# engcang/FAST-LIO-SAM-QN

Hardware: AMD Instinct MI355X
Metric: scan-pair registrations/sec on 100k-pt clouds (higher is better)
Workload: dtype f32 search / f64 accumulate

## Files before the change

### fast-lio-sam-qn_amd/csrc/qn_batch.inc

```

namespace {

template <class F> void lanes_launch(const void* tab, dim3 grid, hipStream_t s) {
  hipLaunchKernelGGL(HIP_KERNEL_NAME(k_lanes<F>), grid, dim3(F::TB), 0, s, (const LaneEntry<typename F::Args>*)tab);
}
template <class A> void lane_push(std::vector<LaneEntry<A>>& v, const A& a, uint32_t nbx) {
  LaneEntry<A> e; memset((void*)&e, 0, sizeof(e)); e.a = a; e.nbx = nbx; v.push_back(e);
}

struct LanePlan {
  qn_ctx* c; size_t off = 0; bool overflow = false; int flush_rc = QN_OK;
  struct Item { void (*fn)(const void*, dim3, hipStream_t); size_t off; dim3 grid; int family; };
  std::vector<Item> items;
  explicit LanePlan(qn_ctx* c_) : c(c_) {}
  template <class F> void add(const std::vector<LaneEntry<typename F::Args>>& e, int family) {
    if (e.empty()) return;
    const size_t bytes = sizeof(LaneEntry<typename F::Args>) * e.size();
    const size_t a = reserve(bytes);
    if (a == SIZE_MAX) return;
    put<F>(e, a, family);
  }
  template <class F, class Fix> void add(std::vector<LaneEntry<typename F::Args>>& e, int family, const void* blob, size_t blob_bytes, Fix fix) {
    if (e.empty()) return;
    const size_t head = (blob_bytes + 255) & ~(size_t)255, bytes = head + sizeof(LaneEntry<typename F::Args>) * e.size();
    const size_t a = reserve(bytes);
    if (a == SIZE_MAX) return;
    memcpy(c->args_h + a, blob, blob_bytes);
    fix(e, (const char*)(c->args_d + a));
    put<F>(e, a + head, family);
  }
  template <class F> void put(const std::vector<LaneEntry<typename F::Args>>& e, size_t a, int family) {
    const size_t bytes = sizeof(LaneEntry<typename F::Args>) * e.size();
    memcpy(c->args_h + a, e.data(), bytes);
    uint32_t gx = 0; for (const auto& x : e) gx = std::max(gx, x.nbx);
    gx = (gx + 7u) & ~7u;
    items.push_back(Item{&lanes_launch<F>, a, dim3(gx, (uint32_t)e.size()), family});
    off = a + bytes;
  }
  size_t reserve(size_t bytes) {
    size_t a = (off + 255) & ~(size_t)255;
    if (a + bytes > c->args_cap) {
      if (items.empty() || bytes > c->args_cap || flush_rc != QN_OK) { overflow = true; return SIZE_MAX; }
      flush_rc = run();
      if (flush_rc == QN_OK && hipStreamSynchronize(c->stream) != hipSuccess) { c->last_error = "batch: stream synchronisation failed while flushing the argument arena"; flush_rc = QN_ERR_HIP; }
      if (flush_rc != QN_OK) { overflow = true; return SIZE_MAX; }
      a = 0;
    }
    return a;
  }
  int run() {
    if (overflow) { if (flush_rc == QN_OK) c->last_error = "batch: argument arena too small for one launch's table"; return QN_ERR_HIP; }
    if (items.empty()) return QN_OK;
    HIPCHK(c, hipMemcpyAsync(c->args_d, c->args_h, off, hipMemcpyHostToDevice, c->stream));
    for (const Item& it : items) { c->prof_begin(it.family, (int)it.grid.y); it.fn(c->args_d + it.off, it.grid, c->stream); c->prof_end(); }
    c->batch_launches += items.size();
    items.clear(); off = 0;
    HIPCHK(c, hipGetLastError());
    return QN_OK;
  }
};

struct ScratchSwap {
  qn_ctx* c;
  static void sw(qn_ctx* c) {
    std::swap(c->scan_sums, c->scan_sums2); std::swap(c->fb_list, c->fb_list2); std::swap(c->big_list, c->big_list2); std::swap(c->fb_count2, c->fb_count2b);
    std::swap(c->knn_idx, c->knn_idx2); std::swap(c->bbox_acc, c->bbox_acc2); std::swap(c->scan_status, c->scan_status2); std::swap(c->staging, c->staging2); std::swap(c->pin_up, c->pin_up2);
  }
  explicit ScratchSwap(qn_ctx* c_) : c(c_) { sw(c); }
  ~ScratchSwap() { sw(c); }
};

struct LaneRun {
  qn_ctx* c = nullptr; uint32_t pair = 0; bool active = false;
  int alias = -1;
  int ticks_left = 0, chunk = 0, chunk_start = 0, next = 0; bool first_chunk = true; long budget = 0;
  bool build_source = true;
};

int lane_set_cloud(qn_ctx* c, int which, const float* xyz, uint32_t n, uint32_t stride, bool on_device, hipStream_t s, GridLaunch* out) {
  CloudBuf& b = c->cloud[which];
  b.n = 0; b.has_grid = b.has_cov = false;
  if (n == 0) return QN_ERR_EMPTY_CLOUD;
  if (!xyz || stride < 12 || (stride & 3)) return QN_ERR_INVALID_ARG;
  if (n > c->max_points) return QN_ERR_CAPACITY;
  const char* dsrc = (const char*)xyz;
  if (!on_device) { const int rc = upload_host_cloud(c, xyz, n, stride, s, &dsrc); if (rc != QN_OK) return rc; }
  b.n = n;
  *out = prep_grid(c, b, dsrc, stride, true);
  return QN_OK;
}

bool batch_supported(const qn_ctx* c) {
  const qn_gicp_params& p = c->params;
  const int maxit = p.force_iterations > 0 ? p.force_iterations : p.max_iterations;
  return c->knob.batch_lanes >= 2 && !c->lanes_failed && maxit > 0 && c->knob.far_enabled && c->knob.knn_hist && !c->knob.verify_track && !c->clk_probe && !c->list_probe && !c->dbg_counters;
}

int lane_args_arena(qn_ctx* c) {
  if (c->args_h) return QN_OK;
  c->args_cap = (size_t)4 << 20;
  HIPCHK(c, hipHostMalloc(&c->args_h, c->args_cap, hipHostMallocDefault));
  HIPCHK(c, hipMalloc(&c->args_d, c->args_cap));
  return QN_OK;
}

int batch_ensure_lanes(qn_ctx* c) {
  HIPCHK(c, hipSetDevice(c->device));
  const int B = std::max(1, std::min(c->knob.batch_lanes, 64));
  if (c->lanes.empty()) c->lanes.push_back(c);
  while ((int)c->lanes.size() < B) {
    qn_ctx* l = nullptr;
    const int rc = (c->knob.fail_lane_create > 0 && (int)c->lanes.size() >= c->knob.fail_lane_create) ? QN_ERR_HIP : ctx_create(c->device, c->max_points, c->stream, &l);
    if (rc != QN_OK) {
      c->last_error = "batch: lane context creation failed (lanes need batch_lanes x the context's device memory)";
      while (c->lanes.size() > 1) { qn_ctx_destroy(c->lanes.back()); c->lanes.pop_back(); }
      (void)hipGetLastError();
      c->lanes_failed = true;
      return rc;
    }
    c->lanes.push_back(l);
  }
  { const int rc = lane_args_arena(c); if (rc != QN_OK) return rc; }
  for (qn_ctx* l : c->lanes) {
    if (l == c) continue;
    if (l->params.k_correspondences != c->params.k_correspondences) l->cloud[0].has_cov = l->cloud[1].has_cov = false;
    l->params = c->params;
    l->lane = c->lane;
  }
  return QN_OK;
}

int batch_register(qn_ctx* owner, const qn_pair_desc* pairs, const uint32_t* idx, uint32_t m, double thr, qn_gicp_result* results, int* valid, int* status,
                   std::vector<const float*>& last_src, std::vector<uint64_t>& last_key, const float* guesses16) {
  hipStream_t s = owner->stream;
  const auto t_call = std::chrono::steady_clock::now();
  const qn_gicp_params& p = owner->params;
  const int k = p.k_correspondences;
  LanePlan plan(owner);
  std::vector<LaneRun> L(m);
  struct AliasGuard {
    std::vector<LaneRun>& L; std::vector<CloudBuf> saved; std::vector<double*> saved_nrm; std::vector<const float*>& last_src;
    AliasGuard(std::vector<LaneRun>& L_, std::vector<const float*>& ls) : L(L_), saved(L_.size()), saved_nrm(L_.size(), nullptr), last_src(ls) {}
    void borrow(size_t l, qn_ctx* from) { qn_ctx* c = L[l].c; saved[l] = c->cloud[0]; saved_nrm[l] = c->nrm_s_sorted; c->cloud[0] = from->cloud[0]; c->nrm_s_sorted = from->nrm_s_sorted; }
    ~AliasGuard() { for (size_t l = 0; l < L.size(); l++) if (L[l].alias >= 0 && saved_nrm[l]) { qn_ctx* c = L[l].c; c->cloud[0] = saved[l]; c->nrm_s_sorted = saved_nrm[l]; c->cloud[0].has_grid = c->cloud[0].has_cov = false; c->cloud[0].n = 0; c->cloud[0].knn_tab = nullptr; last_src[l] = nullptr; } }
  } alias_guard(L, last_src);
  struct FailGuard { std::vector<LaneRun>& L; int* status; bool armed = true; ~FailGuard() { if (armed) for (const LaneRun& R : L) if (R.active) status[R.pair] = QN_ERR_HIP; } } fail_guard{L, status};
  std::vector<LaneEntry<PackBBoxK::Args>> v_pack; std::vector<LaneEntry<CellCountK::Args>> v_count; std::vector<LaneEntry<ScanLookbackK::Args>> v_scan;
  std::vector<LaneEntry<ScatterK::Args>> v_scat; std::vector<LaneEntry<StableCellsK::Args>> v_stab;
// ... 23 lines not shown
      if (R.alias >= 0) { alias_guard.borrow(l, L[R.alias].c); R.build_source = false; }
    }
    int rc = QN_OK; GridLaunch gs, gt;
    if (R.build_source) { last_src[l] = nullptr; rc = lane_set_cloud(c, QN_SOURCE, pd.src, pd.ns, pd.stride_bytes, pd.on_device != 0, s, &gs); }
    if (rc == QN_OK) { ScratchSwap sw(c); rc = lane_set_cloud(c, QN_TARGET, pd.dst, pd.nt, pd.stride_bytes, pd.on_device != 0, s, &gt); }
    if (rc == QN_ERR_HIP) return rc;
    status[R.pair] = rc;
    if (rc != QN_OK) {
      if (R.build_source) { c->cloud[0].has_grid = c->cloud[0].has_cov = false; c->cloud[0].n = 0; }
      c->cloud[1].has_grid = c->cloud[1].has_cov = false; c->cloud[1].n = 0;
      continue;
    }
    if (R.build_source) { push_grid(gs); push_knn(prep_knn(c, c->cloud[0], k, c->knn_idx, nullptr, true)); c->cloud[0].has_cov = true; note_knn_table(c, c->cloud[0], c->knn_idx, k); }
    { ScratchSwap sw(c); push_grid(gt); push_knn(prep_knn(c, c->cloud[1], k, c->knn_idx, nullptr, true)); c->cloud[1].has_cov = true; note_knn_table(c, c->cloud[1], c->knn_idx, k); }
    last_src[l] = R.alias >= 0 ? nullptr : pd.src; last_key[l] = key;
    R.active = true;
  }
  plan.add<PackBBoxK>(v_pack, QN_K_GRID_BUILD); plan.add<CellCountK>(v_count, QN_K_GRID_BUILD); plan.add<ScanLookbackK>(v_scan, QN_K_GRID_BUILD); plan.add<ScatterK>(v_scat, QN_K_GRID_BUILD); plan.add<StableCellsK>(v_stab, QN_K_GRID_BUILD);
  if (k <= 24) {
    if (owner->lane.knn_mm) { plan.add<KnnHistK<false, 32>>(v_sel, QN_K_KNN_SELECT); plan.add<KnnHistK<true, 32>>(v_lst, QN_K_KNN_COV); }
    else { plan.add<KnnHistK<false, 32, false>>(v_sel, QN_K_KNN_SELECT); plan.add<KnnHistK<true, 32, false>>(v_lst, QN_K_KNN_COV); }
  } else {
    if (owner->lane.knn_mm) { plan.add<KnnHistK<false, 48>>(v_sel, QN_K_KNN_SELECT); plan.add<KnnHistK<true, 48>>(v_lst, QN_K_KNN_COV); }
    else { plan.add<KnnHistK<false, 48, false>>(v_sel, QN_K_KNN_SELECT); plan.add<KnnHistK<true, 48, false>>(v_lst, QN_K_KNN_COV); }
  }
  plan.add<KnnSingleK>(v_single, QN_K_KNN_COV);
  if (k <= 16) plan.add<KnnCovK<16, true, 4>>(v_tail, QN_K_KNN_COV); else if (k <= 20) plan.add<KnnCovK<20, true, 4>>(v_tail, QN_K_KNN_COV); else if (k <= 24) plan.add<KnnCovK<24, true, 4>>(v_tail, QN_K_KNN_COV); else plan.add<KnnCovK<32, true, 4>>(v_tail, QN_K_KNN_COV);
  plan.add<CovFromIdxK>(v_cov, QN_K_KNN_COV);

  const int per_outer = p.optimizer == QN_OPT_LM ? 2 : 1;
  const int maxit = p.force_iterations > 0 ? p.force_iterations : p.max_iterations;
  const int fixed_unseeded = fixed_unseeded_iterations(owner) * per_outer;
  const bool exact_ticks = p.force_iterations > 0 && p.optimizer == QN_OPT_GN;
  {
    std::vector<LaneEntry<InitStateK::Args>> v_init; std::vector<float> g16;
    for (LaneRun& R : L) {
      if (!R.active) continue;
      qn_ctx* c = R.c;
      c->gen = 0; c->part_rows = 0; c->far_mode = 2; c->clear_far_now = true; c->unseeded_until = fixed_unseeded; c->count_far_now = false;
      c->result_host->phase = 0;
      R.ticks_left = exact_ticks ? maxit : 1 << 30;
      R.chunk = std::min(fixed_unseeded, R.ticks_left); R.chunk_start = 0; R.next = R.chunk; R.first_chunk = true;
      R.budget = (long)maxit * (p.optimizer == QN_OPT_LM ? (p.lm_max_iterations + 1) : 1) + 2;
      lane_push(v_init, InitStateK::Args{st_cur(c), c->guess_tmp, guesses16 ? 1 : 0, 0, c->far_stats}, 1u);
      if (guesses16) g16.insert(g16.end(), guesses16 + 16 * (size_t)R.pair, guesses16 + 16 * (size_t)R.pair + 16);
    }
    if (!guesses16) plan.add<InitStateK>(v_init, QN_K_SOLVE);
    else
      plan.add<InitStateK>(v_init, QN_K_SOLVE, g16.data(), sizeof(float) * g16.size(), [](std::vector<LaneEntry<InitStateK::Args>>& e, const char* d) {
        for (size_t j = 0; j < e.size(); j++) e[j].a.guess = (const float*)(d + sizeof(float) * 16 * j);
      });
  }
  auto finish_lane = [&](LaneRun& R, int rc) {
    qn_ctx* c = R.c;
    R.active = false;
    status[R.pair] = rc;
    if (rc != QN_OK) return;
    results[R.pair] = c->result_host->r;
    c->trace_len = c->result_host->trace_len; c->aligned_valid = true;
    valid[R.pair] = (results[R.pair].converged && results[R.pair].fitness < thr) ? 1 : 0;
  };
  struct ProfFlush { qn_ctx* c; ~ProfFlush() { c->prof_collect(); } } prof_flush{owner};
  int tick_no = 0;
  for (;;) {
    int stop = 1 << 30; bool any = false;
    for (const LaneRun& R : L) if (R.active) { any = true; stop = std::min(stop, R.next); }
    if (!any) break;
    for (; tick_no < stop; tick_no++) {
      {
        std::vector<LaneEntry<NnSearchArgs>> v_g, v_l; std::vector<LaneEntry<AccumulateK::Args>> v_acc;
        bool group = true, lane = true;
        for (LaneRun& R : L) {
          if (!R.active || tick_no >= R.c->unseeded_until) continue;
          qn_ctx* c = R.c;
          const int t = tick_no - R.chunk_start;
          c->count_far_now = R.first_chunk && (t / per_outer == (R.chunk - 1) / per_outer);
          const NnLaunch N = prep_nn(c, 0, c->sqd, 0);
          group = group && N.group; lane = lane && N.lane;
          lane_push(v_g, N.grid, N.grid_nb); lane_push(v_l, N.list, N.list_nb);
          const uint32_t nb = acc_blocks(c);
          lane_push(v_acc, prep_accumulate(c, 0, true), nb);
          c->count_far_now = false;
        }
        if (lane) plan.add<NnLaneK<0>>(v_g, QN_K_NN_SEARCH); else plan.add<NnSearchK<0, false, QN_NN_BLOCK>>(v_g, QN_K_NN_SEARCH);
        if (group) plan.add<NnSearchK<0, true, QN_BLOCK, true>>(v_l, QN_K_NN_FALLBACK); else plan.add<NnSearchK<0, true, QN_BLOCK>>(v_l, QN_K_NN_FALLBACK);
        plan.add<AccumulateK>(v_acc, QN_K_ACCUMULATE);
      }
      {
        std::vector<LaneEntry<TickArgs>> v_t; std::vector<LaneEntry<FarArgs>> v_f; std::vector<LaneEntry<FarReduceK::Args>> v_r;
        for (LaneRun& R : L) {
          if (!R.active || tick_no < R.c->unseeded_until) continue;
          qn_ctx* c = R.c;
          const TickArgs a = tick_args(c);
          lane_push(v_t, a, tick_blocks(c));
          if (a.far_mode == 1) { lane_push(v_f, far_args(c), (uint32_t)QN_FAR_BLOCKS); lane_push(v_r, far_reduce_args(c), 1u); }
          c->gen++; c->part_rows = -1;
        }
        plan.add<TickK<TICK_TB, 4, 0, false>>(v_t, QN_K_GN_TICK_FUSED); plan.add<FarK>(v_f, QN_K_FAR); plan.add<FarReduceK>(v_r, QN_K_FAR);
      }
    }
    {
      std::vector<LaneEntry<FinalizeK::Args>> v_fin; std::vector<LaneEntry<TickArgs>> v_close; std::vector<LaneEntry<FinalizeFitK::Args>> v_fit;
      for (LaneRun& R : L) {
        if (!R.active || R.next != stop) continue;
        qn_ctx* c = R.c;
        if (exact_ticks && R.ticks_left > R.chunk) lane_push(v_fin, FinalizeK::Args{st_cur(c), c->result_host, c->far_stats}, 1u);
        else {
          const TickArgs a = tick_args(c, 1);
          const uint32_t nb = tick_blocks(c);
          lane_push(v_close, a, nb);
          lane_push(v_fit, FinalizeFitK::Args{st_cur(c), c->result_host, c->far_stats, c->fit_psum, c->fit_pcnt, (int)tick_rows(c)}, 1u);
        }
      }
      plan.add<FinalizeK>(v_fin, QN_K_SOLVE); plan.add<TickK<TICK_TB, 4, 1, false>>(v_close, QN_K_FITNESS); plan.add<FinalizeFitK>(v_fit, QN_K_FITNESS);
    }
    const auto tt0 = std::chrono::steady_clock::now();
    int rc = plan.run();
    if (rc != QN_OK) return rc;
    const auto tt1 = std::chrono::steady_clock::now();
    HIPCHK(owner, hipStreamSynchronize(s));
    if (owner->knob.batch_trace) { const auto tt2 = std::chrono::steady_clock::now();
      fprintf(stderr, "qn batch %p: segment to tick %d  prep+enqueue %.0f us  sync %.0f us  (since call %.0f us)\n", (void*)owner, stop, std::chrono::duration<double, std::micro>(tt1 - tt0).count(),
              std::chrono::duration<double, std::micro>(tt2 - tt1).count(), std::chrono::duration<double, std::micro>(tt2 - t_call).count()); }
    for (LaneRun& R : L) {
      if (!R.active || R.next != stop) continue;
      qn_ctx* c = R.c;
      if (R.first_chunk && (rc = clouds_valid(c)) != QN_OK) { last_src[&R - &L[0]] = nullptr; finish_lane(R, rc); continue; }
      R.budget -= std::max(R.chunk, 1); R.ticks_left -= R.chunk;
      if (c->result_host->phase == 2) { finish_lane(R, QN_OK); continue; }
      if (R.budget <= 0) { c->last_error = "align: device state machine did not terminate"; owner->last_error = c->last_error; finish_lane(R, QN_ERR_HIP); continue; }
      if (R.first_chunk && unseeded_goes_on(c, stop, per_outer, R.ticks_left)) {
        c->unseeded_until = stop + per_outer; R.chunk = per_outer; R.chunk_start = stop; R.next = stop + R.chunk;
        continue;
      }
      const qn::ResultBlock* rb = c->result_host;
      if (R.first_chunk) c->far_mode = rb->far_queries * 16u > c->cloud[0].n ? 1 : 2;
      else c->far_mode = (c->far_mode == 1 ? rb->far_requests : rb->far_misses / (uint32_t)std::max(1, R.chunk)) > 256u ? 1 : 2;
      if (!exact_ticks) R.chunk = R.first_chunk ? TICKS_PER_CHUNK : std::max(2 * per_outer, TICKS_PER_CHUNK / 2);
      else R.chunk = c->far_mode == 1 ? std::min(R.ticks_left, FAR_CHUNK) : R.ticks_left;
      if (R.budget <= 0 || R.chunk <= 0) { c->last_error = "align: device state machine did not terminate"; owner->last_error = c->last_error; finish_lane(R, QN_ERR_HIP); continue; }
      R.first_chunk = false; R.chunk_start = stop; R.next = stop + R.chunk;
    }
  }
  owner->batch_pairs += m;
  fail_guard.armed = false;
  return QN_OK;
}

}

extern "C" int qn_gicp_align_batch_guess(qn_ctx* c, const qn_pair_desc* pairs, const float* guesses16, uint32_t n_pairs, double score_thr, qn_gicp_result* results, int* valid, int* status) {
  if (!c || (n_pairs && (!pairs || !results || !valid || !status))) return QN_ERR_INVALID_ARG;
  if (guesses16)
    for (uint32_t i = 0; i < n_pairs; i++) {
      const float* g = guesses16 + 16 * (size_t)i;
      for (int j = 0; j < 16; j++) if (!std::isfinite(g[j])) { c->last_error = "align_batch_guess: non-finite guess entry"; return QN_ERR_INVALID_ARG; }
      if (g[12] != 0.f || g[13] != 0.f || g[14] != 0.f || g[15] != 1.f) { c->last_error = "align_batch_guess: a guess's last row is not 0 0 0 1"; return QN_ERR_INVALID_ARG; }
    }
  if (n_pairs == 0) return QN_OK;
  HIPCHK(c, hipSetDevice(c->device));
  if (join_target(c) != QN_OK) return QN_ERR_HIP;
  int rc = batch_supported(c) ? batch_ensure_lanes(c) : QN_ERR_NOT_READY;
  if (rc != QN_OK) {
    const bool sp = c->knob.pair_pipeline, sb = c->knob.persist_batch_off; c->knob.pair_pipeline = false; c->knob.persist_batch_off = true;
    for (uint32_t i = 0; i < n_pairs; i++) {
      const qn_pair_desc& p = pairs[i];
// ... 24 lines not shown
```

### fast-lio-sam-qn_amd/csrc/qn_context.h

```cpp
#pragma once
#include <hip/hip_runtime.h>
#include <string>
#include <vector>
#include "qn_gicp_kernels.cuh"

struct CloudBuf {
  uint32_t n = 0, ncells = 0;
  bool has_grid = false, has_cov = false;
  float4* raw = nullptr;
  float4* sorted = nullptr;
  float4* sorted_tmp = nullptr;
  uint32_t* cell_of_pt = nullptr;
  uint32_t* cell_start = nullptr;
  uint32_t* counts = nullptr;
  double* nrm = nullptr;
  qn::GridView grid{};
  qn::GridDims* dims = nullptr;
  qn::GridDims* dims_host = nullptr;
  const int32_t* knn_tab = nullptr; int knn_k = 0;
};

struct ProfSpan { int family; hipEvent_t a, b; int count; };

struct LaneKnobs {
  double cell_override = 0.0;
  int far_group = -1;
  bool far_ranked = true;
  int nn_lane = -1;
  int track_from_tick = 3;
  int knn_mm = 1;
  int knn_trips = 3;
  uint32_t tick_rpb = 2;
};
struct FeatKnobs {
  bool mfma = true;
  int sample = 4;
  bool query_dedupe = false;
  int normals_fg = 0, fpfh_fg = 0;
};
struct OwnKnobs {
  bool device_look = true;
  int single_from_tick = 2;
  bool far_enabled = true;
  int knn_hist = 1;
  bool tgt_early = true;
  bool pair_pipeline = true;
  bool persist = true, prof_persist = false; unsigned long long persist_timeout = 25000000ull;
  bool persist_batch_off = false;
  int batch_lanes = 8;
  int fail_lane_create = 0;
  bool batch_share_source = true;
  bool batch_trace = false;
  int batch_min_share = 4;
  bool c2f_lanes_fpfh = false;
  bool feat_verify = false;
  bool verify_track = false;
};

struct qn_ctx {
  int device = 0;
  uint32_t max_points = 0, max_cells = 0;
  hipStream_t stream = nullptr; bool owns_stream = true;
  LaneKnobs lane; FeatKnobs feat; OwnKnobs knob;
  std::vector<qn_ctx*> lanes; char* args_h = nullptr; char* args_d = nullptr; size_t args_cap = 0; uint64_t batch_launches = 0, batch_pairs = 0; bool is_lane = false;
  bool lanes_failed = false;
  void* slab = nullptr;
  qn_gicp_params params{};
  CloudBuf cloud[2];
  qn::BBoxAcc* bbox_acc = nullptr; qn::BBoxAcc* bbox_acc2 = nullptr;
  unsigned long long* scan_status = nullptr; unsigned long long* scan_status2 = nullptr; uint32_t build_epoch = 0;
  unsigned long long* list_probe = nullptr;
  bool clear_far_now = false;
  char* staging2 = nullptr;
  struct PinZone { char* h = nullptr; hipEvent_t ev = nullptr; bool busy = false; } pin_up, pin_up2;
  char* staging = nullptr;
  uint32_t* scan_sums = nullptr;

  qn::GicpState* state = nullptr;
  uint32_t gen = 0; int part_rows = 0;
  double* partials = nullptr;
  uint32_t* tail_ticket = nullptr;
  double* fit_psum = nullptr; uint32_t* fit_pcnt = nullptr;
  qn_iter_trace* trace = nullptr; uint32_t trace_len = 0;
  int32_t* corr = nullptr; int32_t* nn_idx = nullptr; int32_t* knn_idx = nullptr; float4* nn_ref = nullptr; double* nrm_s_sorted = nullptr; qn::TargetRec* tgt_rec = nullptr; float* sqd = nullptr; float* sqd_fit = nullptr;
  int32_t* far_cand = nullptr; float4* far_cand_ref = nullptr; float2* far_cand_b = nullptr; unsigned long long* far_req = nullptr; uint32_t* far_stats = nullptr; double* far_rows = nullptr; int far_mode = 2;
  uint2* fb_list = nullptr; uint2* big_list = nullptr; uint32_t* fb_count2 = nullptr;
  float4* aligned = nullptr; bool aligned_valid = false;
  double* pose_tmp = nullptr; float* guess_tmp = nullptr;
  qn::ResultBlock* result_host = nullptr; double* scalar_host = nullptr;
  int32_t* dbg_knn_idx = nullptr; float* dbg_knn_d2 = nullptr;
  qn_quatro_params qparams{}; bool qparams_set = false, q_ready = false; double q_last_scale = 1.0;
  float4* q_normals[2] = {nullptr, nullptr}; float* q_spfh[2] = {nullptr, nullptr}; float* q_fpfh_s[2] = {nullptr, nullptr}; float* q_fpfh[2] = {nullptr, nullptr};
  unsigned long long* q_key[2] = {nullptr, nullptr};
  float* q_pair[2] = {nullptr, nullptr}; uint32_t* q_pair_hash[2] = {nullptr, nullptr};
  uint32_t* q_hit = nullptr; uint32_t* q_list = nullptr; uint32_t* q_sel = nullptr; uint2* q_pairs = nullptr; uint32_t* q_counts = nullptr; double* q_T = nullptr;
  void* q_mm_c = nullptr; void* q_mm_q = nullptr; float* q_mm_qn = nullptr; uint32_t* q_mm_L = nullptr; unsigned long long* q_mm_table = nullptr; unsigned long long* q_mm_table_q = nullptr;
  uint32_t q_mm_mask = 0;
  uint2* q_mm_pairs = nullptr; uint32_t* q_mm_cnt = nullptr; uint32_t q_mm_cap = 0, q_mm_ncnt = 0; bool feat_mm_retry = false; double q_wall_ms[3] = {0, 0, 0}; unsigned long long* q_mm_vkeys = nullptr; uint32_t* q_mm_vcnt = nullptr; uint32_t feat_fallbacks = 0, feat_survivors = 0;
  float4* c2f_src = nullptr; float4* c2f_dst = nullptr;
  float* q_mean = nullptr; double* q_mean_psum = nullptr; void* q_host = nullptr;
  int unseeded_until = 3; bool count_far_now = false; int last_extra_unseeded = 0;
  hipStream_t stream2 = nullptr; hipEvent_t ev_pair = nullptr; bool pair_failed = false, tgt_on_stream2 = false, tgt_pending = false, no_pipe = false;
  uint32_t* scan_sums2 = nullptr; uint2* fb_list2 = nullptr; uint2* big_list2 = nullptr; uint32_t* fb_count2b = nullptr; int32_t* knn_idx2 = nullptr;
  unsigned long long* pg_rows = nullptr; unsigned long long* pg_bc = nullptr; unsigned long long* pg_fit = nullptr; uint32_t* pg_status = nullptr; uint32_t* pg_status_host = nullptr;
  unsigned long long* pg_clk = nullptr; uint32_t pg_epoch = 0; bool persist_fits = true; int persist_resident_blocks = 0; uint32_t persist_launches = 0, persist_gave_up = 0;
  uint32_t* dbg_counters = nullptr;
  unsigned long long* clk_probe = nullptr; uint32_t clk_n = 0;
  int32_t* v_corr = nullptr; int32_t* v_nn_idx = nullptr; float* v_sqd = nullptr; float4* v_nn_ref = nullptr; uint32_t* v_counters = nullptr;
  bool prof_on = false, prof_open = false; int prof_depth = 0;
  std::vector<ProfSpan> spans;
  qn_kernel_stat stats[QN_K_COUNT] = {};
  std::string last_error;

  void set_error(const char* what, hipError_t e, int line);
  void prof_begin(int family, int count = 1); void prof_end(); void prof_collect();
  int quatro_normals_width() const { const int g = feat.normals_fg > 0 ? feat.normals_fg : 8; return g >= 16 ? 16 : (g >= 8 ? 8 : 1); }
  int quatro_fpfh_width() const { const int g = feat.fpfh_fg > 0 ? feat.fpfh_fg : 8; return g >= 16 ? 16 : 8; }
};
```

### fast-lio-sam-qn_amd/csrc/qn_device.cuh

```cuda
#pragma once
#include <hip/hip_runtime.h>
#include <stdint.h>
#include "qn_eig3.cuh"
#include "qn_step_math.cuh"

namespace qn {

#define QN_TX 8
#define QN_TY 4
#define QN_TZ 4
#define QN_TILE_CELLS 128

struct GridDims {
  float ox, oy, oz, cell, inv_cell, eps;
  int nx, ny, nz, ntx, nty, ntz;
  uint32_t n;
  uint32_t ncells, nonfinite, pad;
};
struct GridView {
  const float4* pts;
  const uint32_t* cell_start;
  uint32_t* dbg;
  float ox, oy, oz, cell, inv_cell, eps;
  int nx, ny, nz;
// ... 437 lines not shown
  for (uint32_t cb = 0; cb < total; cb += 64) {
    const uint32_t slot = cb + lane;
    const int j = chunk_segment(lds->tile_cid, cb, ex, nxs);
    const uint32_t cnt = min(64u, total - cb);
    wave_lds_fence();
    lds->tile[lane] = slot < total ? g.pts[lds->seg_start[j] + (slot - lds->seg_excl[j])] : make_float4(INF, INF, INF, 0.f);
    lds->tile_cid[lane] = slot < total ? lds->seg_cid[j] : 0xffffffffu;
    wave_lds_fence();
    const uint32_t sub_off = (uint32_t)(S == 1 ? 0 : lane / (64 / S));
    for (uint32_t c = 0; c < cnt; c += 4 * S) {
      float4 cp[4]; uint32_t cc[4];
#pragma unroll
      for (int u = 0; u < 4; u++) { const uint32_t ci = (c + (uint32_t)(S * u) + sub_off) & 63u; cp[u] = lds->tile[ci]; cc[u] = lds->tile_cid[ci]; }
#pragma unroll
      for (int u = 0; u < 4; u++) fn(cp[u], true, cc[u]);
    }
  }
}
template <bool REUSE = false, class Chunks>
__device__ __forceinline__ uint32_t stream_tables(const GridView& g, WaveLds* lds, int ncl, uint32_t nseg_all, Chunks&& chunks, const uint32_t reuse_total = 0) {
  const int lane = threadIdx.x & 63;
  if (REUSE && nseg_all <= 64u) { chunks(reuse_total); return reuse_total; }
  uint32_t ncand = 0;
  for (uint32_t sb = 0; sb < nseg_all; sb += 64) {
    const uint32_t sidx = sb + lane;
    uint32_t s = 0, len = 0, scid = 0;
    if (sidx < nseg_all) {
      int c = 0;
#pragma unroll
      for (int step = 32; step > 0; step >>= 1) { const int t = c + step; if (t < ncl && lds->cl_seg0[t] <= sidx) c = t; }
      const int* b = lds->box[c];
      const int x0 = b[0], x1 = b[1], y0 = b[2], y1 = b[3], z0 = b[4];
      const int tx0 = x0 >> 3, ntr = (x1 >> 3) - tx0 + 1;
      const int li = (int)(sidx - lds->cl_seg0[c]);
      int t, rr; divmod_small(li, ntr, rr, t);
      if (lds->cl_tile_mode[c]) {
        const int ty0 = y0 >> 2, ntyr = (y1 >> 2) - ty0 + 1;
        int qz_, ry_; divmod_small(rr, ntyr, qz_, ry_);
        const uint32_t tile = ((uint32_t)((z0 >> 2) + qz_) * g.nty + (ty0 + ry_)) * g.ntx + (tx0 + t);
        s = g.cell_start[tile << 7]; len = g.cell_start[(tile + 1) << 7] - s;
      } else {
        const int nyr = y1 - y0 + 1;
        int qz_, ry_; divmod_small(rr, nyr, qz_, ry_);
        const int ry = y0 + ry_, rz = z0 + qz_, tx = tx0 + t;
        const int xa = max(x0, tx << 3), xb = min(x1, (tx << 3) + 7);
        const uint32_t k0 = cell_key(g, xa, ry, rz);
        s = g.cell_start[k0]; len = g.cell_start[k0 + (xb - xa) + 1] - s;
      }
      scid = (uint32_t)c;
    }
    const uint32_t incl = wave_incl_scan_u32(len, lane);
    const uint32_t total = rdlane(incl, 63);
    if (total == 0) continue;
    wave_lds_fence();
    lds->seg_excl[lane] = incl - len; lds->seg_start[lane] = s; lds->seg_cid[lane] = scid;
    wave_lds_fence();
    chunks(total);
    ncand += total;
  }
  return ncand;
}
template <int S, bool REUSE = false, class Fn>
__device__ __forceinline__ uint32_t stream_clusters(const GridView& g, WaveLds* lds, int ncl, uint32_t nseg_all, Fn&& fn, const uint32_t reuse_total = 0) {
  return stream_tables<REUSE>(g, lds, ncl, nseg_all, [&](const uint32_t total) __attribute__((always_inline)) { stream_chunks<S>(g, lds, total, fn); }, reuse_total);
}

template <int S, class Sink>
__device__ __forceinline__ bool wave_search(const GridView& g, float qx, float qy, float qz, bool active, float& r, const float r_cap,
                                            int max_rounds, Sink& sink, WaveLds* lds, float& d_unseen) {
  const int lane = threadIdx.x & 63;
  const int cx = cell_coord(qx, g.ox, g.inv_cell, g.nx);
  const int cy = cell_coord(qy, g.oy, g.inv_cell, g.ny);
  const int cz = cell_coord(qz, g.oz, g.inv_cell, g.nz);
  bool certified = false;
  unsigned long long todo = __ballot(active);
  for (int round = 0; todo != 0 && round < max_rounds; round++) {
    const bool mine = (todo >> lane) & 1ull;
    uint32_t cid; int ncl; uint32_t nseg_all;
    build_clusters<S>(g, lds, todo, cx, cy, cz, qx, qy, qz, r, cid, ncl, nseg_all);
    const uint32_t ncand = stream_clusters<S>(g, lds, ncl, nseg_all, [&](const float4& cp, bool in_tile, uint32_t ccid) __attribute__((always_inline)) {
      sink.consider(mine && in_tile && ccid == cid, sqdist(qx, qy, qz, cp.x, cp.y, cp.z), __float_as_uint(cp.w));
    });
    sink.template finish<S>(mine);
    if (g.dbg && lane == 0) { atomicAdd(&g.dbg[0], (uint32_t)ncl); atomicAdd(&g.dbg[1], ncand); }
    bool retry = false;
    if (mine) {
      const int* b = lds->box[cid];
      const int ex0 = b[0], ex1 = b[1], ey0 = b[2], ey1 = b[3], ez0 = b[4], ez1 = b[5];
      const float INF = __int_as_float(0x7f800000);
      float d = INF;
      if (ex0 > 0) d = fminf(d, qx - (g.ox + ex0 * g.cell));
      if (ex1 < g.nx - 1) d = fminf(d, (g.ox + (ex1 + 1) * g.cell) - qx);
      if (ey0 > 0) d = fminf(d, qy - (g.oy + ey0 * g.cell));
      if (ey1 < g.ny - 1) d = fminf(d, (g.oy + (ey1 + 1) * g.cell) - qy);
      if (ez0 > 0) d = fminf(d, qz - (g.oz + ez0 * g.cell));
      if (ez1 < g.nz - 1) d = fminf(d, (g.oz + (ez1 + 1) * g.cell) - qz);
      if (d == INF || !(r == r)) { certified = true; d_unseen = INF; }
      else { d -= g.eps; d_unseen = d; certified = d > 0.f && sink.full() && sink.worst_d2() < d * d; }
      if (!certified) {
        if (sink.full()) r = fmaxf(sqrtf(sink.worst_d2()) * 1.000001f + g.eps, r + g.eps);
        else {
          const int f = sink.found();
          r = f > 0 ? fmaxf(r * sqrtf((float)sink.wanted() / (float)f) * 1.25f, r + g.cell) : 2.f * r + g.cell;
        }
        r = fminf(r, r_cap);
        if (round + 1 < max_rounds) { retry = true; sink.reset(); }
      }
    }
    todo = __ballot(retry);
    if (g.dbg && lane == 0 && todo) atomicAdd(&g.dbg[3], (uint32_t)__popcll(todo));
  }
  return certified;
}

struct CapBox {
  float o2[3];
  float S;
};
__device__ __forceinline__ CapBox cap_of(const GridView& g, float qx, float qy, float qz) {
  CapBox c;
  const float ox = fmaxf(fmaxf(g.ox - qx, qx - (g.ox + g.nx * g.cell)), 0.f);
  const float oy = fmaxf(fmaxf(g.oy - qy, qy - (g.oy + g.ny * g.cell)), 0.f);
  const float oz = fmaxf(fmaxf(g.oz - qz, qz - (g.oz + g.nz * g.cell)), 0.f);
  c.o2[0] = ox * ox; c.o2[1] = oy * oy; c.o2[2] = oz * oz; c.S = (c.o2[0] + c.o2[1]) + c.o2[2];
  return c;
}
__device__ __forceinline__ float cap_extent(const GridView& g, const CapBox& c, float r, int axis) {
  const float rest = c.S - c.o2[axis];
  if (rest <= 0.f) return r;
  const float v = r * r - rest * 0.999999f;
  return v > 0.f ? sqrtf(v) * 1.000001f + g.eps : g.eps;
}
__device__ __forceinline__ float cap_face_dist(const CapBox& c, float f, int axis) {
  const float rest = (c.S - c.o2[axis]) * 0.999999f;
  return rest > 0.f ? sqrtf(f * f + rest) * 0.999999f : f;
}

struct SingleStats { uint32_t rounds, cand, segs; float r_first, r_last; };
__device__ __forceinline__ void wave_search_single(const GridView& g, float qx, float qy, float qz, float r, const float r_cap,
                                                   unsigned long long& best_out, float& second_out, float& d_unseen, WaveLds* lds, SingleStats& st_out, const bool stats) {
  const int lane = threadIdx.x & 63;
  const float INF = __int_as_float(0x7f800000);
  const CapBox cap = cap_of(g, qx, qy, qz);
  if (cap.S > 0.f) r = fminf(fmaxf(r, sqrtf(cap.S) + g.cell), fmaxf(r_cap, r));
  if (stats) { st_out.rounds = 0; st_out.cand = 0; st_out.segs = 0; st_out.r_first = r; }
  float done2 = -1.f;
  int ptx0 = 0, ptx1 = -1, pty0 = 0, pty1 = -1, ptz0 = 0, ptz1 = -1;
  unsigned long long best = QN_INF_KEY; float second = INF;
  for (int round = 0;; round++) {
    const float rx = cap_extent(g, cap, r, 0), ry = cap_extent(g, cap, r, 1), rz = cap_extent(g, cap, r, 2);
    int x0 = rfl(cell_coord(qx - rx, g.ox, g.inv_cell, g.nx)), x1 = rfl(cell_coord(qx + rx, g.ox, g.inv_cell, g.nx));
    int y0 = rfl(cell_coord(qy - ry, g.oy, g.inv_cell, g.ny)), y1 = rfl(cell_coord(qy + ry, g.oy, g.inv_cell, g.ny));
    int z0 = rfl(cell_coord(qz - rz, g.oz, g.inv_cell, g.nz)), z1 = rfl(cell_coord(qz + rz, g.oz, g.inv_cell, g.nz));
    const int tx0 = x0 >> 3, ntr = (x1 >> 3) - tx0 + 1;
    int nseg = ntr * (y1 - y0 + 1) * (z1 - z0 + 1);
    const bool tile_mode = nseg > 128;
    int ty0 = 0, ntyr = 1;
    if (tile_mode) {
      x0 = (x0 >> 3) << 3; x1 = min(((x1 >> 3) << 3) + 7, g.nx - 1);
      y0 = (y0 >> 2) << 2; y1 = min(((y1 >> 2) << 2) + 3, g.ny - 1);
      z0 = (z0 >> 2) << 2; z1 = min(((z1 >> 2) << 2) + 3, g.nz - 1);
      ty0 = y0 >> 2; ntyr = (y1 >> 2) - ty0 + 1;
      nseg = ntr * ntyr * ((z1 >> 2) - (z0 >> 2) + 1);
    }
    const int nyr = y1 - y0 + 1;
    if (!tile_mode || done2 < 0.f) { best = QN_INF_KEY; second = INF; done2 = -1.f; }
    const float in2 = r * r * 1.000002f;
// ... 205 lines not shown
```

### fast-lio-sam-qn_amd/csrc/qn_engine.hip

```cpp
#include <hip/hip_runtime.h>
#include <cfloat>
#include <cmath>
#include <cstdio>
#include <cstring>
#include <string>
#include <vector>
#include <atomic>
#include <thread>
#include <chrono>
#include "qn_instances.h"
#include "qn_context.h"
#include "qn_selftest.cuh"
#include "qn_pool.h"
#include "qn_kf_internal.h"

using namespace qn;

#define HIPCHK(ctx, call)                                                                 \
  do { hipError_t e_ = (call);                                                            \
       if (e_ != hipSuccess) { (ctx)->set_error(#call, e_, __LINE__); return QN_ERR_HIP; } \
  } while (0)

void qn_ctx::set_error(const char* what, hipError_t e, int line) {
  char buf[512]; snprintf(buf, sizeof(buf), "%s -> %s (qn_engine.hip:%d)", what, hipGetErrorString(e), line);
// ... 30 lines not shown
    case QN_OK: return "ok"; case QN_ERR_INVALID_ARG: return "invalid argument"; case QN_ERR_EMPTY_CLOUD: return "empty cloud";
    case QN_ERR_CAPACITY: return "cloud exceeds context capacity"; case QN_ERR_NOT_READY: return "clouds/covariances not set";
    case QN_ERR_HIP: return "HIP runtime error"; case QN_ERR_NO_DEVICE: return "no gfx950 device (no CPU fallback)";
    case QN_ERR_INTERNAL: return "internal error (a bounded loop left its bound)";
  }
  return "unknown status";
}
extern "C" const char* qn_last_error(const qn_ctx* ctx) { return ctx ? ctx->last_error.c_str() : "null context"; }

extern "C" void qn_gicp_default_params(qn_gicp_params* p) {
  if (!p) return;
  memset(p, 0, sizeof(*p));
  p->k_correspondences = 20; p->max_iterations = 64; p->max_corr_dist = (double)FLT_MAX;
  p->transformation_epsilon = 5e-4; p->rotation_epsilon = 2e-3; p->optimizer = QN_OPT_LM;
  p->lm_max_iterations = 10; p->lm_init_lambda_factor = 1e-9; p->force_iterations = 0;
  p->ransac_iterations = 0; p->ransac_outlier_threshold = 0.05; p->euclidean_fitness_epsilon = -DBL_MAX;
}

struct Slab {
  char* base = nullptr; size_t off = 0, cap = 0;
  template <class T> void take(T*& p, size_t bytes) {
    const size_t a = (off + 255) & ~(size_t)255;
    if (base) p = (T*)(base + a);
    off = a + bytes;
  }
};
static void carve_cloud(qn_ctx* c, Slab& sl, CloudBuf& b) {
  sl.take(b.raw, sizeof(float4) * c->max_points);
  sl.take(b.sorted, sizeof(float4) * c->max_points);
  sl.take(b.sorted_tmp, sizeof(float4) * c->max_points);
  sl.take(b.cell_of_pt, sizeof(uint32_t) * c->max_points);
  sl.take(b.cell_start, sizeof(uint32_t) * ((size_t)c->max_cells + 1));
  sl.take(b.counts, sizeof(uint32_t) * ((size_t)c->max_cells + 1));
  sl.take(b.nrm, sizeof(double) * 3 * c->max_points);
  sl.take(b.dims, sizeof(GridDims));
}

static int ctx_create(int device, uint32_t max_points, hipStream_t shared_stream, qn_ctx** out);
extern "C" int qn_ctx_create(int device, uint32_t max_points, qn_ctx** out) { return ctx_create(device, max_points, nullptr, out); }
static int ctx_create(int device, uint32_t max_points, hipStream_t shared_stream, qn_ctx** out) {
  if (!out || max_points == 0) return QN_ERR_INVALID_ARG;
  *out = nullptr;
  if (max_points > QN_CTX_MAX_POINTS) return QN_ERR_CAPACITY;
  int ndev = 0;
  if (hipGetDeviceCount(&ndev) != hipSuccess || ndev <= 0 || device < 0 || device >= ndev) return QN_ERR_NO_DEVICE;
  qn_ctx* c = new qn_ctx();
  c->device = device; c->max_points = max_points;
  size_t mc = (size_t)max_points * 16; if (mc < (1u << 18)) mc = 1u << 18; if (mc > (1u << 23)) mc = 1u << 23;
  c->max_cells = (uint32_t)mc;
  qn_gicp_default_params(&c->params);
  int rc = QN_OK;
  auto fail = [&](int code) { qn_ctx_destroy(c); return code; };
  if (hipSetDevice(device) != hipSuccess) return fail(QN_ERR_NO_DEVICE);
  if (shared_stream) { c->stream = shared_stream; c->owns_stream = false; c->is_lane = true; }
  else if (hipStreamCreateWithFlags(&c->stream, hipStreamNonBlocking) != hipSuccess) return fail(QN_ERR_HIP);
#define CA(call) if ((call) != hipSuccess) return fail(QN_ERR_HIP)
  auto carve = [&](Slab& sl) {
    carve_cloud(c, sl, c->cloud[0]);
    carve_cloud(c, sl, c->cloud[1]);
    sl.take(c->staging, (size_t)max_points * 32);
    sl.take(c->scan_sums, sizeof(uint32_t) * (c->max_cells / (QN_BLOCK * QN_SCAN_ITEMS) + 2));
    sl.take(c->state, 2 * sizeof(GicpState));
    sl.take(c->partials, 2 * sizeof(double) * (QN_ACC_MAX_BLOCKS + 8) * QN_NPART);
    sl.take(c->nn_idx, sizeof(int32_t) * max_points);
    sl.take(c->knn_idx, sizeof(int32_t) * (size_t)max_points * 32);
    sl.take(c->nn_ref, sizeof(float4) * max_points);
    sl.take(c->nrm_s_sorted, sizeof(double) * 3 * max_points);
    sl.take(c->tgt_rec, sizeof(TargetRec) * max_points);
    sl.take(c->fit_psum, sizeof(double) * (QN_ACC_MAX_BLOCKS + 8));
    sl.take(c->fit_pcnt, sizeof(uint32_t) * (QN_ACC_MAX_BLOCKS + 8));
    sl.take(c->trace, sizeof(qn_iter_trace) * QN_MAX_TRACE);
    sl.take(c->corr, sizeof(int32_t) * max_points);
    sl.take(c->sqd, sizeof(float) * max_points);
    sl.take(c->sqd_fit, sizeof(float) * max_points);
    sl.take(c->far_cand, sizeof(int32_t) * QN_FAR_M * (size_t)max_points);
    sl.take(c->far_cand_ref, sizeof(float4) * max_points);
    sl.take(c->far_cand_b, sizeof(float2) * max_points);
    sl.take(c->far_req, sizeof(unsigned long long) * (max_points / 64 + 2));
    sl.take(c->far_stats, 4 * sizeof(uint32_t));
    sl.take(c->far_rows, sizeof(double) * QN_FAR_BLOCKS * QN_NPART);
    sl.take(c->fb_list, sizeof(uint2) * max_points);
    sl.take(c->big_list, sizeof(uint2) * max_points);
    sl.take(c->fb_count2, 4 * sizeof(uint32_t));
    sl.take(c->aligned, sizeof(float4) * max_points);
    sl.take(c->pose_tmp, sizeof(double) * 16);
    sl.take(c->guess_tmp, sizeof(float) * 16);
    sl.take(c->scan_sums2, sizeof(uint32_t) * (c->max_cells / (QN_BLOCK * QN_SCAN_ITEMS) + 2));
    sl.take(c->fb_list2, sizeof(uint2) * max_points);
    sl.take(c->big_list2, sizeof(uint2) * max_points);
    sl.take(c->fb_count2b, 4 * sizeof(uint32_t));
    sl.take(c->knn_idx2, sizeof(int32_t) * (size_t)max_points * 32);
    sl.take(c->staging2, (size_t)max_points * 32);
    sl.take(c->bbox_acc, 2 * (QN_BBOX_MAX_BLOCKS + 1) * sizeof(BBoxAcc)); c->bbox_acc2 = c->bbox_acc ? c->bbox_acc + (QN_BBOX_MAX_BLOCKS + 1) : nullptr;
    sl.take(c->scan_status, sizeof(unsigned long long) * 2 * (c->max_cells / (QN_BLOCK * QN_SCAN_ITEMS) + 2)); c->scan_status2 = c->scan_status ? c->scan_status + (c->max_cells / (QN_BLOCK * QN_SCAN_ITEMS) + 2) : nullptr;
    sl.take(c->pg_rows, sizeof(unsigned long long) * 3 * QN_PERSIST_ROWS * QN_PERSIST_RSTRIDE);
    sl.take(c->pg_bc, sizeof(unsigned long long) * 64);
    sl.take(c->pg_fit, sizeof(unsigned long long) * (QN_PERSIST_MAX_BLOCKS + 1) * 4);
    sl.take(c->pg_status, 4 * sizeof(uint32_t));
    sl.take(c->tail_ticket, 4 * sizeof(uint32_t));
  };
  { Slab dry; carve(dry);
    Slab sl; sl.cap = (dry.off + ((size_t)2 << 20) - 1) & ~(((size_t)2 << 20) - 1);
    CA(hipMalloc(&c->slab, sl.cap)); sl.base = (char*)c->slab; carve(sl); }
  CA(hipMemsetAsync(c->far_stats, 0, 4 * sizeof(uint32_t), c->stream));
  CA(hipHostMalloc(&c->result_host, sizeof(ResultBlock), hipHostMallocDefault));
  for (int w = 0; w < 2; w++) { CA(hipHostMalloc(&c->cloud[w].dims_host, sizeof(GridDims), hipHostMallocDefault)); memset(c->cloud[w].dims_host, 0, sizeof(GridDims)); }
  CA(hipHostMalloc(&c->scalar_host, 64 * sizeof(double), hipHostMallocDefault));
  CA(hipHostMalloc(&c->pg_status_host, 4 * sizeof(uint32_t), hipHostMallocDefault));
  CA(hipMemsetAsync(c->pg_rows, 0xFF, sizeof(unsigned long long) * 3 * QN_PERSIST_ROWS * QN_PERSIST_RSTRIDE, c->stream));
  CA(hipMemsetAsync(c->pg_bc, 0, sizeof(unsigned long long) * 64, c->stream));
  CA(hipMemsetAsync(c->pg_fit, 0, sizeof(unsigned long long) * (QN_PERSIST_MAX_BLOCKS + 1) * 4, c->stream));
  CA(hipMemsetAsync(c->pg_status, 0, 4 * sizeof(uint32_t), c->stream));
  CA(hipMemsetAsync(c->tail_ticket, 0, 4 * sizeof(uint32_t), c->stream));
  CA(hipMemsetAsync(c->state, 0, 2 * sizeof(GicpState), c->stream));
  hipLaunchKernelGGL(k_bbox_acc_init, dim3(1), dim3(256), 0, c->stream, c->bbox_acc, 2 * (QN_BBOX_MAX_BLOCKS + 1));
  CA(hipMemsetAsync(c->fb_count2, 0, 4 * sizeof(uint32_t), c->stream)); CA(hipMemsetAsync(c->fb_count2b, 0, 4 * sizeof(uint32_t), c->stream));
  CA(hipMemsetAsync(c->scan_status, 0, sizeof(unsigned long long) * 2 * (c->max_cells / (QN_BLOCK * QN_SCAN_ITEMS) + 2), c->stream));
  for (int w = 0; w < 2; w++) CA(hipMemsetAsync(c->cloud[w].counts, 0, sizeof(uint32_t) * ((size_t)c->max_cells + 1), c->stream));
  CA(hipMemsetAsync(c->knn_idx, 0xff, sizeof(int32_t) * (size_t)max_points * 32, c->stream));
  if (c->knn_idx2) CA(hipMemsetAsync(c->knn_idx2, 0xff, sizeof(int32_t) * (size_t)max_points * 32, c->stream));
  CA(hipStreamSynchronize(c->stream));
#undef CA
  {
    int per_cu = 0; hipDeviceProp_t prop;
    if (hipOccupancyMaxActiveBlocksPerMultiprocessor(&per_cu, reinterpret_cast<const void*>(&k_align_persist<QN_PERSIST_TB, false>), QN_PERSIST_TB, 0) != hipSuccess || hipGetDeviceProperties(&prop, device) != hipSuccess) { (void)hipGetLastError(); per_cu = 0; prop.multiProcessorCount = 0; }
    c->persist_resident_blocks = per_cu * prop.multiProcessorCount;
    c->persist_fits = c->persist_resident_blocks >= QN_PERSIST_MAX_BLOCKS + 1;
  }
  *out = c;
  return QN_OK;
}

extern "C" void qn_ctx_destroy(qn_ctx* c) {
  if (!c) return;
  hipSetDevice(c->device);
  if (c->stream) hipStreamSynchronize(c->stream);
  if (c->stream2) hipStreamSynchronize(c->stream2);
  for (qn_ctx* l : c->lanes) if (l != c) qn_ctx_destroy(l);
  c->lanes.clear();
  if (c->args_h) hipHostFree(c->args_h);
  hipFree(c->args_d);
  c->prof_collect();
  hipFree(c->slab);
  hipFree(c->q_mm_c); hipFree(c->q_mm_q); hipFree(c->q_mm_qn); hipFree(c->q_mm_L); hipFree(c->q_mm_table); hipFree(c->q_mm_table_q); hipFree(c->q_mm_pairs); hipFree(c->q_mm_cnt); hipFree(c->q_mm_vkeys); hipFree(c->q_mm_vcnt);
  for (int w = 0; w < 2; w++) { hipFree(c->q_normals[w]); hipFree(c->q_spfh[w]); hipFree(c->q_fpfh_s[w]); hipFree(c->q_fpfh[w]); hipFree(c->q_key[w]); hipFree(c->q_pair[w]); hipFree(c->q_pair_hash[w]); }
  hipFree(c->q_hit); hipFree(c->q_list); hipFree(c->q_sel); hipFree(c->q_pairs); hipFree(c->q_counts); hipFree(c->q_T); hipFree(c->q_mean); hipFree(c->q_mean_psum);
  if (c->q_host) hipHostFree(c->q_host);
  hipFree(c->c2f_src); hipFree(c->c2f_dst);
  hipFree(c->dbg_knn_idx); hipFree(c->dbg_knn_d2); hipFree(c->dbg_counters);
  hipFree(c->v_corr); hipFree(c->v_nn_idx); hipFree(c->v_sqd); hipFree(c->v_nn_ref); hipFree(c->v_counters);
  if (c->result_host) hipHostFree(c->result_host);
  for (int w = 0; w < 2; w++) if (c->cloud[w].dims_host) hipHostFree(c->cloud[w].dims_host);
  if (c->scalar_host) hipHostFree(c->scalar_host);
  hipFree(c->pg_clk); if (c->list_probe) hipFree(c->list_probe); if (c->pg_status_host) hipHostFree(c->pg_status_host);
  if (c->ev_pair) hipEventDestroy(c->ev_pair);
  for (qn_ctx::PinZone* z : {&c->pin_up, &c->pin_up2}) { if (z->ev) hipEventDestroy(z->ev); if (z->h) hipHostFree(z->h); }
  if (c->stream2) { hipStreamSynchronize(c->stream2); hipStreamDestroy(c->stream2); }
  if (c->stream && c->owns_stream) hipStreamDestroy(c->stream);
  delete c;
}

static int clouds_valid(qn_ctx* c);
extern "C" void* qn_ctx_stream(qn_ctx* c) { return c ? (void*)c->stream : nullptr; }
int qn_ctx_int_device(const qn_ctx* c) { return c->device; }
int qn_ctx_int_max_points(const qn_ctx* c) { return (int)c->max_points; }
extern "C" int qn_ctx_synchronize(qn_ctx* c) {
  if (!c) return QN_ERR_INVALID_ARG;
  HIPCHK(c, hipStreamSynchronize(c->stream));
  if (c->stream2) HIPCHK(c, hipStreamSynchronize(c->stream2));
  c->prof_collect();
  return clouds_valid(c);
}

extern "C" int qn_gicp_set_params(qn_ctx* c, const qn_gicp_params* p) {
  if (!c || !p) return QN_ERR_INVALID_ARG;
  if (p->k_correspondences < 1 || p->k_correspondences > 32 || p->max_iterations < 0 || p->lm_max_iterations < 1 ||
      (p->optimizer != QN_OPT_LM && p->optimizer != QN_OPT_GN) || !(p->max_corr_dist > 0) || !(p->lm_init_lambda_factor >= 0)) return QN_ERR_INVALID_ARG;
  if (p->k_correspondences != c->params.k_correspondences) { c->cloud[0].has_cov = c->cloud[1].has_cov = false; }
  c->params = *p;
  return QN_OK;
}

extern "C" int qn_gicp_get_params(const qn_ctx* c, qn_gicp_params* p) { if (!c || !p) return QN_ERR_INVALID_ARG; *p = c->params; return QN_OK; }

static GicpConfig make_cfg(const qn_ctx* c) {
  GicpConfig g; const qn_gicp_params& p = c->params;
  g.k = p.k_correspondences; g.max_iterations = p.max_iterations; g.optimizer = p.optimizer; g.lm_max_iterations = p.lm_max_iterations;
  g.force_iterations = p.force_iterations; g.max_corr_dist_sq = p.max_corr_dist * p.max_corr_dist;
  g.transformation_epsilon = p.transformation_epsilon; g.rotation_epsilon = p.rotation_epsilon; g.lm_init_lambda_factor = p.lm_init_lambda_factor;
  return g;
}

static inline GicpState* st_cur(qn_ctx* c) { return c->state + (c->gen & 1u); }
static inline GicpState* st_nxt(qn_ctx* c) { return c->state + ((c->gen + 1u) & 1u); }
static inline double* part_cur(qn_ctx* c) { return c->partials + (size_t)(c->gen & 1u) * (QN_ACC_MAX_BLOCKS + 8) * QN_NPART; }
static inline double* part_nxt(qn_ctx* c) { return c->partials + (size_t)((c->gen + 1u) & 1u) * (QN_ACC_MAX_BLOCKS + 8) * QN_NPART; }

static bool pair_pipeline_ready(qn_ctx* c) {
  if (c->stream2) return true;
  if (c->pair_failed || !c->knn_idx2) return false;
  const bool ok = hipStreamCreateWithFlags(&c->stream2, hipStreamNonBlocking) == hipSuccess && hipEventCreateWithFlags(&c->ev_pair, hipEventDisableTiming) == hipSuccess;
  if (!ok) { c->pair_failed = true; if (c->stream2) { hipStreamDestroy(c->stream2); c->stream2 = nullptr; } (void)hipGetLastError(); }
  return ok;
}
static void swap_scratch(qn_ctx* c) {
  std::swap(c->stream, c->stream2); std::swap(c->scan_sums, c->scan_sums2); std::swap(c->fb_list, c->fb_list2); std::swap(c->big_list, c->big_list2);
  std::swap(c->fb_count2, c->fb_count2b); std::swap(c->knn_idx, c->knn_idx2);
  std::swap(c->bbox_acc, c->bbox_acc2); std::swap(c->scan_status, c->scan_status2);
  std::swap(c->pin_up, c->pin_up2);
  std::swap(c->staging, c->staging2);
}
struct TargetScope {
  qn_ctx* c; bool on;
  TargetScope(qn_ctx* c_, bool on_) : c(c_), on(on_) { if (on) swap_scratch(c); }
  ~TargetScope() { if (on) { (void)hipEventRecord(c->ev_pair, c->stream); swap_scratch(c); c->tgt_pending = true; } }
};
static int join_target(qn_ctx* c) {
  if (!c->tgt_pending) return QN_OK;
  c->tgt_pending = false;
  return hipStreamWaitEvent(c->stream, c->ev_pair, 0) == hipSuccess ? QN_OK : QN_ERR_HIP;
}

struct GridLaunch { PackBBoxK::Args pack; uint32_t pack_nb; CellCountK::Args count; ScanLookbackK::Args scan; uint32_t scan_nb; ScatterK::Args scat; StableCellsK::Args stab; uint32_t nb; };
static GridLaunch prep_grid(qn_ctx* c, CloudBuf& b, const char* dsrc, uint32_t stride, bool lanes = false) {
  const uint32_t n = b.n;
  GridView& g = b.grid;
  memset(&g, 0, sizeof(g));
  g.pts = b.sorted; g.cell_start = b.cell_start; g.dbg = c->dbg_counters; g.n = n; g.dims = b.dims;
  GridLaunch L;
  L.nb = (n + QN_BLOCK - 1) / QN_BLOCK;
  L.scan_nb = (c->max_cells + QN_BLOCK * QN_SCAN_ITEMS - 1) / (QN_BLOCK * QN_SCAN_ITEMS);
  if (((++c->build_epoch) & 0x3fffffffu) == 0u) ++c->build_epoch;
  constexpr int LONE_PACK_BLOCKS = 64;
  static_assert(LONE_PACK_BLOCKS <= QN_BBOX_MAX_BLOCKS, "the accumulator has one box per block");
  L.pack_nb = std::min<uint32_t>(L.nb, (uint32_t)(lanes ? QN_BBOX_MAX_BLOCKS : LONE_PACK_BLOCKS));
  L.pack = PackBBoxK::Args{dsrc, stride, n, b.raw, c->bbox_acc, c->max_cells, c->lane.cell_override, b.dims, b.dims_host};
  L.count = CellCountK::Args{b.raw, n, g, b.counts, b.cell_of_pt};
  L.scan = ScanLookbackK::Args{b.counts, b.dims, b.cell_start, c->scan_status, c->build_epoch, n};
  L.scat = ScatterK::Args{b.raw, n, b.cell_of_pt, b.cell_start, b.counts, b.sorted_tmp};
  L.stab = StableCellsK::Args{b.sorted_tmp, n, b.cell_of_pt, b.cell_start, b.sorted};
  b.has_grid = true; b.has_cov = false; b.knn_tab = nullptr;
  return L;
}
static int build_grid(qn_ctx* c, CloudBuf& b, const char* dsrc, uint32_t stride) {
  hipStream_t s = c->stream;
  const GridLaunch L = prep_grid(c, b, dsrc, stride);
  { ProfScope ps(c, QN_K_GRID_BUILD);
    hipLaunchKernelGGL(k_pack_bbox_dims, dim3(L.pack_nb), dim3(QN_BLOCK), 0, s, L.pack.in, L.pack.stride, L.pack.n, L.pack.raw, L.pack.acc, L.pack.max_cells, L.pack.cell_override, L.pack.dims_dev, L.pack.dims_host);
    hipLaunchKernelGGL(k_cell_count, dim3(L.nb), dim3(QN_BLOCK), 0, s, L.count.pts, L.count.n, L.count.g, L.count.counts, L.count.cell_of_pt);
    hipLaunchKernelGGL(k_scan_lookback, dim3(L.scan_nb), dim3(QN_BLOCK), 0, s, L.scan.in, L.scan.dims, L.scan.out, L.scan.status, L.scan.epoch, L.scan.total);
    hipLaunchKernelGGL(k_scatter, dim3(L.nb), dim3(QN_BLOCK), 0, s, L.scat.pts, L.scat.n, L.scat.cell_of_pt, L.scat.cell_start, L.scat.counts, L.scat.sorted);
    hipLaunchKernelGGL(k_stable_cells, dim3(L.nb), dim3(QN_BLOCK), 0, s, L.stab.in, L.stab.n, L.stab.cell_of_pt, L.stab.cell_start, L.stab.out); }
  HIPCHK(c, hipGetLastError());
  return QN_OK;
}
static int clouds_valid(qn_ctx* c) {
  for (int w = 0; w < 2; w++)
    if (c->cloud[w].has_grid && c->cloud[w].dims_host && c->cloud[w].dims_host->nonfinite) {
      c->last_error = w == 0 ? "source cloud contains non-finite coordinates (is_dense == false clouds are not supported)" : "target cloud contains non-finite coordinates (is_dense == false clouds are not supported)";
      c->cloud[w].has_grid = c->cloud[w].has_cov = false;
      return QN_ERR_INVALID_ARG;
    }
  return QN_OK;
}

static int upload_host_cloud(qn_ctx* c, const float* xyz, uint32_t n, uint32_t& stride, hipStream_t s, const char** dsrc) {
  hipPointerAttribute_t at;
  const bool pinned = hipPointerGetAttributes(&at, xyz) == hipSuccess && at.type == hipMemoryTypeHost;
  if (!pinned) (void)hipGetLastError();
  if (pinned) {
    if (stride <= 32) { HIPCHK(c, hipMemcpyAsync(c->staging, xyz, (size_t)(n - 1) * stride + 12, hipMemcpyHostToDevice, s)); }
    else { HIPCHK(c, hipMemcpy2DAsync(c->staging, 16, xyz, stride, 16, n, hipMemcpyHostToDevice, s)); stride = 16; }
    *dsrc = (const char*)c->staging;
    return QN_OK;
  }
  qn_ctx::PinZone& z = c->pin_up;
  if (!z.h) { HIPCHK(c, hipHostMalloc((void**)&z.h, (size_t)c->max_points * 16, hipHostMallocDefault)); HIPCHK(c, hipEventCreateWithFlags(&z.ev, hipEventDisableTiming)); }
  if (z.busy) { HIPCHK(c, hipEventSynchronize(z.ev)); z.busy = false; }
  float* o = (float*)z.h; const char* in = (const char*)xyz;
  for (uint32_t i = 0; i < n; i++, in += stride, o += 3) { const float* p = (const float*)in; o[0] = p[0]; o[1] = p[1]; o[2] = p[2]; }
  HIPCHK(c, hipMemcpyAsync(c->staging, z.h, (size_t)n * 12, hipMemcpyHostToDevice, s));
  HIPCHK(c, hipEventRecord(z.ev, s)); z.busy = true;
  stride = 12; *dsrc = (const char*)c->staging;
  return QN_OK;
}

static int set_cloud(qn_ctx* c, int which, const float* xyz, uint32_t n, uint32_t stride, bool on_device) {
  if (!c || (which != 0 && which != 1)) return QN_ERR_INVALID_ARG;
  CloudBuf& b = c->cloud[which];
  b.n = 0; b.has_grid = b.has_cov = false;
// ... 33 lines not shown
  L.single_nb = std::min<uint32_t>((b.n + 3) / 4, lanes ? 128 : 2048);
  L.single = KnnSingleK::Args{b.grid, k, kidx, kd2, c->big_list, genc, c->fb_list, c->fb_count2 + 2};
  L.tail_nb = std::min<uint32_t>((b.n + 63) / 64, lanes ? 64 : 1024);
  L.tail = KnnCovArgs{b.grid, b.raw, k, r0, 64, b.nrm, kidx, kd2, c->fb_list, c->fb_count2 + 2};
  L.cov_nb = (b.n + QN_BLOCK - 1) / QN_BLOCK;
  L.cov = CovFromIdxK::Args{b.raw, b.sorted, b.n, k, kidx, b.nrm, &b == &c->cloud[0] ? c->nrm_s_sorted : (double*)nullptr, &b == &c->cloud[0] ? (TargetRec*)nullptr : c->tgt_rec, c->fb_count2};
  return L;
}
template <int KMAX>
static void launch_knn_cov(qn_ctx* c, CloudBuf& b, int k, int32_t* kidx, float* kd2) {
  hipStream_t s = c->stream;
  if (c->knob.knn_hist) {
    const KnnLaunch L = prep_knn(c, b, k, kidx, kd2);
    constexpr int HCAP = KMAX <= 24 ? 32 : 48;
    { ProfScope sel(c, QN_K_KNN_SELECT);
      if (!c->lane.knn_mm) hipLaunchKernelGGL(HIP_KERNEL_NAME(k_knn_hist<false, HCAP, false>), dim3(L.sel_nb), dim3(QN_KNN_BLOCK), 0, s, L.sel.g, L.sel.k, L.sel.r0, L.sel.max_rounds, L.sel.knn_idx, L.sel.knn_d2, L.sel.fb_list, L.sel.fb_count, L.sel.gen_list, L.sel.gen_count);
      else hipLaunchKernelGGL(HIP_KERNEL_NAME(k_knn_hist<false, HCAP>), dim3(L.sel_nb), dim3(QN_KNN_BLOCK), 0, s, L.sel.g, L.sel.k, L.sel.r0, L.sel.max_rounds, L.sel.knn_idx, L.sel.knn_d2, L.sel.fb_list, L.sel.fb_count, L.sel.gen_list, L.sel.gen_count); }
    ProfScope ps(c, QN_K_KNN_COV);
    if (!c->lane.knn_mm) hipLaunchKernelGGL(HIP_KERNEL_NAME(k_knn_hist<true, HCAP, false>), dim3(L.lst_nb), dim3(QN_KNN_BLOCK), 0, s, L.lst.g, L.lst.k, L.lst.r0, L.lst.max_rounds, L.lst.knn_idx, L.lst.knn_d2, L.lst.fb_list, L.lst.fb_count, L.lst.gen_list, L.lst.gen_count);
    else hipLaunchKernelGGL(HIP_KERNEL_NAME(k_knn_hist<true, HCAP>), dim3(L.lst_nb), dim3(QN_KNN_BLOCK), 0, s, L.lst.g, L.lst.k, L.lst.r0, L.lst.max_rounds, L.lst.knn_idx, L.lst.knn_d2, L.lst.fb_list, L.lst.fb_count, L.lst.gen_list, L.lst.gen_count);
    hipLaunchKernelGGL(k_knn_single, dim3(L.single_nb), dim3(QN_BLOCK), 0, s, L.single.g, L.single.k, L.single.knn_idx, L.single.knn_d2, L.single.list, L.single.count, L.single.gen_list, L.single.gen_count);
    hipLaunchKernelGGL(HIP_KERNEL_NAME(k_knn_cov<KMAX, true, 4>), dim3(L.tail_nb), dim3(QN_BLOCK), 0, s, L.tail.g, L.tail.raw, L.tail.k, L.tail.r0, L.tail.max_rounds, L.tail.cov, L.tail.knn_idx, L.tail.knn_d2, L.tail.fb_list, L.tail.fb_count);
    hipLaunchKernelGGL(k_cov_from_idx, dim3(L.cov_nb), dim3(QN_BLOCK), 0, s, L.cov.raw, L.cov.sorted, L.cov.n, L.cov.k, L.cov.knn_idx, L.cov.nrm, L.cov.nrm_sorted, L.cov.rec, L.cov.list_counts);
    return;
  }
  const float r0 = knn_first_radius(b);
  ProfScope ps(c, QN_K_KNN_COV);
  {
    const uint32_t nb = (b.n + QN_BLOCK / 4 - 1) / (QN_BLOCK / 4);
    hipLaunchKernelGGL(HIP_KERNEL_NAME(k_knn_cov<KMAX, false, 4>), dim3(nb), dim3(QN_BLOCK), 0, s, b.grid, b.raw, k, r0, 2, b.nrm, kidx, kd2, c->fb_list, c->fb_count2);
  }
  hipLaunchKernelGGL(HIP_KERNEL_NAME(k_knn_cov<KMAX, true, 4>), dim3(std::min<uint32_t>((b.n + 63) / 64, 512)), dim3(QN_BLOCK), 0, s, b.grid, b.raw, k, r0, 64, b.nrm, kidx, kd2, c->fb_list, c->fb_count2);
  const uint32_t nbp = (b.n + QN_BLOCK - 1) / QN_BLOCK;
  hipLaunchKernelGGL(k_cov_from_idx, dim3(nbp), dim3(QN_BLOCK), 0, s, b.raw, b.sorted, b.n, k, kidx, b.nrm,
                     &b == &c->cloud[0] ? c->nrm_s_sorted : (double*)nullptr, &b == &c->cloud[0] ? (TargetRec*)nullptr : c->tgt_rec, c->fb_count2);
}
static void note_knn_table(qn_ctx* c, CloudBuf& b, const int32_t* kidx, int k) {
  for (CloudBuf& o : c->cloud) if (&o != &b && o.knn_tab == kidx) o.knn_tab = nullptr;
  b.knn_tab = kidx; b.knn_k = k;
}
static int compute_cov(qn_ctx* c, int which, int32_t* kidx, float* kd2) {
  if (!c || (which != 0 && which != 1)) return QN_ERR_INVALID_ARG;
  CloudBuf& b = c->cloud[which];
  if (!b.has_grid) return b.n == 0 ? QN_ERR_EMPTY_CLOUD : QN_ERR_NOT_READY;
  HIPCHK(c, hipSetDevice(c->device));
  const int k = c->params.k_correspondences;
  const bool on2 = which == QN_TARGET && c->tgt_on_stream2 && !c->prof_on && kidx == c->knn_idx && c->stream2 != nullptr;
  if (which == QN_TARGET && !on2 && join_target(c) != QN_OK) return QN_ERR_HIP;
  if (on2) kidx = c->knn_idx2;
  TargetScope scope(c, on2);
  if (k <= 16) launch_knn_cov<16>(c, b, k, kidx, kd2);
  else if (k <= 20) launch_knn_cov<20>(c, b, k, kidx, kd2);
  else if (k <= 24) launch_knn_cov<24>(c, b, k, kidx, kd2);
  else launch_knn_cov<32>(c, b, k, kidx, kd2);
  HIPCHK(c, hipGetLastError());
  b.has_cov = true;
  if (kidx == c->knn_idx || kidx == c->knn_idx2) note_knn_table(c, b, kidx, k);
  return QN_OK;
}
extern "C" int qn_gicp_compute_covariances(qn_ctx* c, int which) { return compute_cov(c, which, c->knn_idx, nullptr); }

constexpr float NN_R0 = -1.f;
constexpr float NN_BIG_RATIO = 2.5f;
constexpr int NN_BIG_BLOCKS = 4096; constexpr uint32_t NN_FB_BLOCKS = 512;
struct NnLaunch { NnSearchArgs grid; uint32_t grid_nb; NnSearchArgs list; uint32_t list_nb; bool group; bool lane; };
static NnLaunch prep_nn(qn_ctx* c, int mode , float* sqd_out, int cond) {
  CloudBuf &S = c->cloud[0], &T = c->cloud[1];
  const uint32_t nb = (S.n + QN_NN_BLOCK / 4 - 1) / (QN_NN_BLOCK / 4);
  const uint32_t nb4 = (S.n + QN_BLOCK / 4 - 1) / (QN_BLOCK / 4);
  const double thr2 = c->params.max_corr_dist * c->params.max_corr_dist;
  GicpState* st = st_cur(c);
  uint32_t* fbc = &st->fb_count; uint32_t* bgc = &st->big_count;
  uint32_t* far_stats = (mode == 0 && c->count_far_now) ? c->far_stats : nullptr;
  int big_blocks = NN_BIG_BLOCKS;
  const uint32_t fbb = std::min<uint32_t>(nb4, NN_FB_BLOCKS);
  NnOpt opt; opt.clear_ref = (mode == 0 && c->clear_far_now) ? c->far_cand_ref : nullptr; opt.cond = cond;
  const bool batch = c->knob.persist_batch_off;
  opt.group = c->lane.far_group >= 0 ? c->lane.far_group : (batch ? 2048 : 0); opt.group_min = 0;
  if (mode == 0 && opt.group > 0) big_blocks = std::min(big_blocks, std::max(64, (opt.group + QN_BLOCK / 64 - 1) / (QN_BLOCK / 64)));
  opt.probe = mode == 0 ? c->list_probe : nullptr;
  constexpr uint32_t LIST_SMALL = 6000;
  opt.fb_small = (mode == 0 && !c->knob.persist_batch_off) ? LIST_SMALL : 0u;
  NnOpt opt0; opt0.clear_ref = nullptr; opt0.cond = 0; opt0.group = 0; opt0.group_min = 0; opt0.probe = nullptr; opt0.fb_small = 0;
  if (mode == 0) c->clear_far_now = false;
  const NnOpt& o = mode == 0 ? opt : opt0;
  NnLaunch L;
  L.lane = (c->lane.nn_lane > 0 || (c->lane.nn_lane < 0 && c->knob.persist_batch_off)) && mode == 0;
  L.grid_nb = L.lane ? (S.n + 255u) / 256u : nb; L.list_nb = fbb + (uint32_t)big_blocks; L.group = mode == 0 && opt.group > 0;
  L.grid = NnSearchArgs{S.grid, T.grid, st, thr2, NN_R0, 1, c->corr, sqd_out, c->nn_idx, c->nn_ref, c->fb_list, fbc, c->big_list, bgc, 0, NN_BIG_RATIO, far_stats, o};
  L.list = NnSearchArgs{S.grid, T.grid, st, thr2, NN_R0, 64, c->corr, sqd_out, c->nn_idx, c->nn_ref, c->fb_list, fbc, c->big_list, bgc, big_blocks, NN_BIG_RATIO, far_stats, o};
  return L;
}
#define QN_NN_ARGS(A) A.src, A.tgt, A.st, A.thr2, A.r0, A.max_rounds, A.corr, A.sqd, A.nn_idx, A.nn_ref, A.fb_list, A.fb_count, A.big_list, A.big_count, A.big_blocks, A.big_ratio, A.far_stats, A.opt
static void enqueue_nn(qn_ctx* c, int mode , float* sqd_out, int cond = 0) {
  hipStream_t s = c->stream;
  const NnLaunch L = prep_nn(c, mode, sqd_out, cond);
  if (L.grid.opt.probe) (void)hipMemsetAsync(c->list_probe, 0, sizeof(unsigned long long) * 4 * 16384, s);
  const NnSearchArgs& G = L.grid; const NnSearchArgs& F = L.list;
  if (mode == 0) {
    { ProfScope ps(c, QN_K_NN_SEARCH);
      if (L.lane) hipLaunchKernelGGL(HIP_KERNEL_NAME(k_nn_lane<0>), dim3(L.grid_nb), dim3(256), 0, s, G);
      else hipLaunchKernelGGL(HIP_KERNEL_NAME(k_nn_search<0, false, QN_NN_BLOCK>), dim3(L.grid_nb), dim3(QN_NN_BLOCK), 0, s, QN_NN_ARGS(G)); }
    { ProfScope ps(c, QN_K_NN_FALLBACK);
      if (L.group) hipLaunchKernelGGL(HIP_KERNEL_NAME(k_nn_search<0, true, QN_BLOCK, true>), dim3(L.list_nb), dim3(QN_BLOCK), 0, s, QN_NN_ARGS(F));
      else hipLaunchKernelGGL(HIP_KERNEL_NAME(k_nn_search<0, true, QN_BLOCK>), dim3(L.list_nb), dim3(QN_BLOCK), 0, s, QN_NN_ARGS(F)); }
  } else {
    ProfScope ps(c, QN_K_FITNESS);
    hipLaunchKernelGGL(HIP_KERNEL_NAME(k_nn_search<1, false, QN_NN_BLOCK>), dim3(L.grid_nb), dim3(QN_NN_BLOCK), 0, s, QN_NN_ARGS(G));
    hipLaunchKernelGGL(HIP_KERNEL_NAME(k_nn_search<1, true, QN_BLOCK>), dim3(L.list_nb), dim3(QN_BLOCK), 0, s, QN_NN_ARGS(F));
  }
}
static void enqueue_verify(qn_ctx* c) {
  hipStream_t s = c->stream;
  CloudBuf &S = c->cloud[0], &T = c->cloud[1];
  const uint32_t nb = (S.n + QN_NN_BLOCK / 4 - 1) / (QN_NN_BLOCK / 4), nb4 = (S.n + QN_BLOCK / 4 - 1) / (QN_BLOCK / 4);
  const double thr2 = c->params.max_corr_dist * c->params.max_corr_dist;
  GicpState* st = st_cur(c);
  uint32_t* fbc = &st->fb_count; uint32_t* bgc = &st->big_count;
  hipLaunchKernelGGL(k_reset_lists, dim3(1), dim3(64), 0, s, st);
  hipLaunchKernelGGL(HIP_KERNEL_NAME(k_nn_search<0, false, QN_NN_BLOCK>), dim3(nb), dim3(QN_NN_BLOCK), 0, s, S.grid, T.grid, st, thr2, NN_R0, 1, c->v_corr, c->v_sqd, c->v_nn_idx, c->v_nn_ref, c->fb_list, fbc, c->big_list, bgc, 0, NN_BIG_RATIO, (uint32_t*)nullptr, NnOpt{nullptr, 0, 0, 0, nullptr, 0});
  hipLaunchKernelGGL(HIP_KERNEL_NAME(k_nn_search<0, true, QN_BLOCK>), dim3(std::min<uint32_t>(nb4, NN_FB_BLOCKS) + NN_BIG_BLOCKS), dim3(QN_BLOCK), 0, s, S.grid, T.grid, st, thr2, NN_R0, 64, c->v_corr, c->v_sqd, c->v_nn_idx, c->v_nn_ref, c->fb_list, fbc, c->big_list, bgc, NN_BIG_BLOCKS, NN_BIG_RATIO, (uint32_t*)nullptr, NnOpt{nullptr, 0, 0, 0, nullptr, 0});
  hipLaunchKernelGGL(k_verify_nn, dim3((S.n + 255) / 256), dim3(256), 0, s, S.n, st, c->nn_idx, c->v_nn_idx, (const float*)nullptr, c->v_sqd, c->corr, c->v_corr, c->v_counters);
  hipLaunchKernelGGL(k_reset_lists, dim3(1), dim3(64), 0, s, st);
}
static uint32_t acc_blocks(const qn_ctx* c) { return std::min<uint32_t>((c->cloud[0].n + QN_BLOCK - 1) / QN_BLOCK, QN_ACC_MAX_BLOCKS); }
constexpr uint32_t TICK_TB = 512;
static_assert(TICK_TB == QN_PERSIST_TB, "k_align_persist reads the tracking records k_tick leaves: one block shape");
static uint32_t tick_ppt(const qn_ctx* c) { return std::max<uint32_t>(1u, (c->cloud[0].n + TICK_TB * QN_ACC_MAX_BLOCKS - 1) / (TICK_TB * QN_ACC_MAX_BLOCKS)); }
static uint32_t tick_rows(const qn_ctx* c) { const uint32_t per = TICK_TB * tick_ppt(c); return (c->cloud[0].n + per - 1) / per; }
static uint32_t tick_rpb(const qn_ctx* c) { return c->knob.persist_batch_off ? std::max(1u, c->lane.tick_rpb) : 1u; }
static uint32_t tick_blocks(const qn_ctx* c) { const uint32_t rpb = tick_rpb(c); return (tick_rows(c) + rpb - 1) / rpb; }
static TailArgs tail_args(qn_ctx* c, int enabled, int rows, const LookArgs* look = nullptr) {
  TailArgs t; memset(&t, 0, sizeof(t));
  t.st_in = st_cur(c); t.st_out = st_nxt(c); t.cfg = make_cfg(c); t.trace = c->trace; t.ticket = c->tail_ticket; t.enabled = enabled; t.rows = rows;
  if (look) t.look = *look;
  return t;
}
static AccumulateK::Args prep_accumulate(qn_ctx* c, int cond, bool tail, const LookArgs* look = nullptr) {
  CloudBuf &S = c->cloud[0];
  const AccumulateK::Args a{S.raw, S.n, S.nrm, c->tgt_rec, c->corr, st_cur(c), part_cur(c), cond, tail_args(c, tail ? 1 : 0, (int)acc_blocks(c), look)};
  if (tail) { c->gen++; c->part_rows = -1; } else c->part_rows = (int)acc_blocks(c);
  return a;
}
static void enqueue_accumulate(qn_ctx* c, int cond, bool tail, const LookArgs* look = nullptr) {
  ProfScope ps(c, QN_K_ACCUMULATE);
  const uint32_t nb = acc_blocks(c);
  const AccumulateK::Args a = prep_accumulate(c, cond, tail, look);
  hipLaunchKernelGGL(k_accumulate, dim3(nb), dim3(QN_BLOCK), 0, c->stream, a);
}
static SolveArgs prep_solve(qn_ctx* c, int mode, int will_produce, const LookArgs* look) {
  LookArgs la; memset(&la, 0, sizeof(la)); if (look) la = *look;
  const SolveArgs a{st_cur(c), st_nxt(c), part_cur(c), c->part_rows, make_cfg(c), c->trace, mode, will_produce, la};
  c->gen++; c->part_rows = -1;
  return a;
}
static void enqueue_solve(qn_ctx* c, int mode, int will_produce, const LookArgs* look = nullptr) {
  ProfScope ps(c, QN_K_SOLVE);
  const SolveArgs a = prep_solve(c, mode, will_produce, look);
  hipLaunchKernelGGL(HIP_KERNEL_NAME(k_solve<TICK_TB>), dim3(1), dim3(TICK_TB), 0, c->stream, a.st_in, a.st_out, a.partials, a.rows, a.cfg, a.trace, a.mode, a.will_produce, a.look);
}
static TickArgs tick_args(qn_ctx* c, int mode = 0) {
  CloudBuf &S = c->cloud[0], &T = c->cloud[1];
  TickArgs a;
  a.src = S.grid; a.tgt = T.grid; a.part_out = part_cur(c);
  a.thr2 = c->params.max_corr_dist * c->params.max_corr_dist;
  a.nn_idx = c->nn_idx; a.nn_ref = c->nn_ref; a.nrm_s = c->nrm_s_sorted; a.tgt_rec = c->tgt_rec; a.ppt = tick_ppt(c); a.rpb = tick_rpb(c); a.rows = tick_rows(c);
  a.far_mode = c->knob.far_enabled ? c->far_mode : 0; a.tgt_raw = T.raw; a.cand = c->far_cand; a.cand_ref = c->far_cand_ref; a.cand_b = c->far_cand_b; a.far_req = c->far_req; a.far_stats = c->far_stats;
  a.tail = tail_args(c, (mode == 0 && a.far_mode != 1) ? 1 : 0, (int)tick_rows(c));
  a.aligned = c->aligned; a.fit_psum = c->fit_psum; a.fit_pcnt = c->fit_pcnt;
  a.clk = c->clk_probe ? c->clk_probe + 8 * (c->clk_n++ % 256) : nullptr; a.clk_blk = c->clk_probe ? c->clk_probe + 8 * 256 : nullptr;
  return a;
// ... 459 lines not shown
  c->params.k_correspondences = ksave;
  b.has_cov = had && (k == ksave);
  if (rc != QN_OK) return rc;
  HIPCHK(c, hipMemcpyAsync(idx_out, c->dbg_knn_idx, sizeof(int32_t) * (size_t)b.n * k, hipMemcpyDeviceToHost, c->stream));
  HIPCHK(c, hipMemcpyAsync(d2_out, c->dbg_knn_d2, sizeof(float) * (size_t)b.n * k, hipMemcpyDeviceToHost, c->stream));
  HIPCHK(c, hipStreamSynchronize(c->stream));
  c->prof_collect();
  return clouds_valid(c);
}

extern "C" int qn_gicp_linearize(qn_ctx* c, const double T[16], double H[36], double b6[6], double* err, int32_t* corr_out, float* sqd_out) {
  if (c && join_target(c) != QN_OK) return QN_ERR_HIP;
  int rc = ready(c); if (rc != QN_OK) return rc;
  if (!T || !H || !b6 || !err) return QN_ERR_INVALID_ARG;
  HIPCHK(c, hipSetDevice(c->device));
  hipStream_t s = c->stream;
  HIPCHK(c, hipMemcpyAsync(c->pose_tmp, T, sizeof(double) * 16, hipMemcpyHostToDevice, s));
  hipLaunchKernelGGL(k_set_pose, dim3(1), dim3(64), 0, s, st_cur(c), c->pose_tmp, 0, 0);
  enqueue_nn(c, 0, c->sqd); enqueue_accumulate(c, 0, false); enqueue_solve(c, 1, 0);
  GicpState* hs = (GicpState*)malloc(sizeof(GicpState));
  hipError_t e = hipMemcpyAsync(hs, st_cur(c), sizeof(GicpState), hipMemcpyDeviceToHost, s);
  if (e == hipSuccess && corr_out) e = hipMemcpyAsync(corr_out, c->corr, sizeof(int32_t) * c->cloud[0].n, hipMemcpyDeviceToHost, s);
  if (e == hipSuccess && sqd_out) e = hipMemcpyAsync(sqd_out, c->sqd, sizeof(float) * c->cloud[0].n, hipMemcpyDeviceToHost, s);
  if (e == hipSuccess) e = hipStreamSynchronize(s);
  if (e != hipSuccess) { free(hs); c->set_error("linearize readback", e, __LINE__); return QN_ERR_HIP; }
  memcpy(H, hs->H, sizeof(double) * 36); memcpy(b6, hs->b, sizeof(double) * 6); *err = hs->y0;
  free(hs);
  c->prof_collect();
  return clouds_valid(c);
}

extern "C" int qn_gicp_compute_error(qn_ctx* c, const double T[16], double* err) {
  if (c && join_target(c) != QN_OK) return QN_ERR_HIP;
  int rc = ready(c); if (rc != QN_OK) return rc;
  if (!T || !err) return QN_ERR_INVALID_ARG;
  HIPCHK(c, hipSetDevice(c->device));
  hipStream_t s = c->stream;
  HIPCHK(c, hipMemcpyAsync(c->pose_tmp, T, sizeof(double) * 16, hipMemcpyHostToDevice, s));
  hipLaunchKernelGGL(k_set_pose, dim3(1), dim3(64), 0, s, st_cur(c), c->pose_tmp, 1, 1);
  enqueue_accumulate(c, 0, false); enqueue_solve(c, 2, 0);
  HIPCHK(c, hipMemcpyAsync(c->scalar_host, &st_cur(c)->yi, sizeof(double), hipMemcpyDeviceToHost, s));
  HIPCHK(c, hipStreamSynchronize(s));
  *err = c->scalar_host[0];
  c->prof_collect();
  return clouds_valid(c);
}

extern "C" int qn_prof_enable(qn_ctx* c, int on) { if (!c) return QN_ERR_INVALID_ARG; c->prof_on = on != 0; return QN_OK; }
extern "C" int qn_prof_reset(qn_ctx* c) { if (!c) return QN_ERR_INVALID_ARG; c->prof_collect(); for (auto& s : c->stats) { s.total_ms = 0; s.launches = 0; } return QN_OK; }
extern "C" int qn_prof_get(qn_ctx* c, int fam, qn_kernel_stat* out) {
  if (!c || !out || fam < 0 || fam >= QN_K_COUNT) return QN_ERR_INVALID_ARG;
  c->prof_collect(); *out = c->stats[fam]; return QN_OK;
}
extern "C" int qn_debug_set(qn_ctx* c, const char* key, double v) {
  if (!c || !key) return QN_ERR_INVALID_ARG;
  std::string k(key);
  if (k == "cell") { c->lane.cell_override = v; c->cloud[0].has_grid = c->cloud[1].has_grid = false; }
  else if (k == "device_look") c->knob.device_look = v != 0;
  else if (k == "far_group") c->lane.far_group = (int)v;
  else if (k == "tgt_early") c->knob.tgt_early = v != 0;
  else if (k == "c2f_lanes_fpfh") c->knob.c2f_lanes_fpfh = v != 0;
  else if (k == "normals_fg") c->feat.normals_fg = (int)v;
  else if (k == "fpfh_fg") c->feat.fpfh_fg = (int)v;
  else if (k == "far_ranked") c->lane.far_ranked = v != 0;
  else if (k == "pair_pipeline") c->knob.pair_pipeline = v != 0;
  else if (k == "persist") c->knob.persist = v != 0;
  else if (k == "persist_timeout") c->knob.persist_timeout = v < 1 ? 1ull : (unsigned long long)v;
  else if (k == "prof_persist") c->knob.prof_persist = v != 0;
  else if (k == "persist_probe") {
    if (v != 0 && !c->pg_clk) { if (hipMalloc(&c->pg_clk, 8 * (64 * 16 + 16)) != hipSuccess) return QN_ERR_HIP; }
    if (c->pg_clk) (void)hipMemset(c->pg_clk, 0, 8 * (64 * 16 + 16));
    if (v == 0) { (void)hipFree(c->pg_clk); c->pg_clk = nullptr; }
  }
  else if (k == "batch_lanes") {
    const int b = std::max(1, std::min((int)v, 64));
    if (b < (int)c->lanes.size()) { if (hipStreamSynchronize(c->stream) != hipSuccess) return QN_ERR_HIP; while ((int)c->lanes.size() > std::max(b, 1)) { qn_ctx* l = c->lanes.back(); c->lanes.pop_back(); if (l != c) qn_ctx_destroy(l); } }
    c->knob.batch_lanes = b; c->lanes_failed = false;
  }
  else if (k == "fail_lane_create") c->knob.fail_lane_create = (int)v;
  else if (k == "batch_share_source") c->knob.batch_share_source = v != 0;
  else if (k == "batch_trace") c->knob.batch_trace = v != 0;
  else if (k == "batch_member") c->knob.persist_batch_off = v != 0;
  else if (k == "knn_hist") c->knob.knn_hist = v != 0;
  else if (k == "nn_lane") c->lane.nn_lane = v < 0 ? -1 : (v != 0 ? 1 : 0);
  else if (k == "track_from_tick") c->lane.track_from_tick = v < 1 ? 1 : (int)v;
  else if (k == "single_from_tick") c->knob.single_from_tick = v < 1 ? 1 : (int)v;
  else if (k == "knn_trips") c->lane.knn_trips = v < 1 ? 1 : (int)v;
  else if (k == "knn_mm") c->lane.knn_mm = v != 0;
  else if (k == "dbg_counters") {
    if (v != 0 && !c->dbg_counters) { if (hipMalloc(&c->dbg_counters, 16 * sizeof(uint32_t)) != hipSuccess) return QN_ERR_HIP; }
    if (c->dbg_counters) (void)hipMemset(c->dbg_counters, 0, 16 * sizeof(uint32_t));
    if (v == 0) { (void)hipFree(c->dbg_counters); c->dbg_counters = nullptr; }
    for (int w = 0; w < 2; w++) c->cloud[w].grid.dbg = c->dbg_counters;
  }
  else if (k == "far") c->knob.far_enabled = v != 0;
  else if (k == "feat_mfma") c->feat.mfma = v != 0;
  else if (k == "feat_sample") c->feat.sample = (int)v;
  else if (k == "feat_query_dedupe") c->feat.query_dedupe = v != 0;
  else if (k == "feat_verify") { c->knob.feat_verify = v != 0; if (c->q_mm_vcnt) (void)hipMemset(c->q_mm_vcnt, 0, 16); }
  else if (k == "list_probe") {
    if (v != 0 && !c->list_probe) { if (hipMalloc(&c->list_probe, sizeof(unsigned long long) * 4 * 16384) != hipSuccess) return QN_ERR_HIP; }
    if (v == 0 && c->list_probe) { (void)hipFree(c->list_probe); c->list_probe = nullptr; }
  }
  else if (k == "clk_probe") {
    if (v != 0 && !c->clk_probe) { if (hipMalloc(&c->clk_probe, 8 * 8 * 256 + 8 * 12 * 1024) != hipSuccess) return QN_ERR_HIP; }
    if (c->clk_probe) (void)hipMemset(c->clk_probe, 0, 8 * 8 * 256 + 8 * 12 * 1024);
    c->clk_n = 0; if (v == 0) { (void)hipFree(c->clk_probe); c->clk_probe = nullptr; }
  }
  else if (k == "tick_rpb") c->lane.tick_rpb = v < 1 ? 1u : (uint32_t)v;
  else if (k == "batch_min_share") c->knob.batch_min_share = v < 1 ? 1 : (int)v;
  else if (k == "verify_track") {
    if (v != 0 && !c->v_counters) {
      const size_t n = c->max_points;
      if (hipMalloc(&c->v_corr, 4 * n) != hipSuccess || hipMalloc(&c->v_nn_idx, 4 * n) != hipSuccess || hipMalloc(&c->v_sqd, 4 * n) != hipSuccess ||
          hipMalloc(&c->v_nn_ref, 16 * n) != hipSuccess || hipMalloc(&c->v_counters, 16) != hipSuccess) return QN_ERR_HIP;
    }
    if (c->v_counters) (void)hipMemset(c->v_counters, 0, 16);
    c->knob.verify_track = v != 0;
  }
  else return QN_ERR_INVALID_ARG;
  return QN_OK;
}
extern "C" int qn_debug_selftest(qn_ctx* c, uint32_t n_waves, uint32_t seed, uint32_t* mismatches) {
  if (!c || !mismatches || n_waves == 0 || n_waves > 65536) return QN_ERR_INVALID_ARG;
  HIPCHK(c, hipSetDevice(c->device));
  std::vector<uint32_t> h((size_t)n_waves * 128);
  uint64_t x = 0x9e3779b97f4a7c15ull ^ seed;
  for (auto& v : h) { x ^= x << 13; x ^= x >> 7; x ^= x << 17; v = (uint32_t)(x >> 16); }
  uint32_t* d = nullptr;
  HIPCHK(c, hipMalloc(&d, (h.size() + 1) * sizeof(uint32_t)));
  int rc = QN_OK; uint32_t bad = 0xffffffffu;
  if (hipMemcpyAsync(d, h.data(), h.size() * sizeof(uint32_t), hipMemcpyHostToDevice, c->stream) != hipSuccess || hipMemsetAsync(d + h.size(), 0, sizeof(uint32_t), c->stream) != hipSuccess) rc = QN_ERR_HIP;
  if (rc == QN_OK) {
    hipLaunchKernelGGL(k_selftest_wave, dim3(n_waves), dim3(64), 0, c->stream, d, d + (size_t)n_waves * 64, d + h.size());
    if (hipMemcpyAsync(&bad, d + h.size(), sizeof(uint32_t), hipMemcpyDeviceToHost, c->stream) != hipSuccess || hipStreamSynchronize(c->stream) != hipSuccess) rc = QN_ERR_HIP;
  }
  (void)hipFree(d);
  if (rc != QN_OK) { c->last_error = "selftest: HIP call failed"; return rc; }
  *mismatches = bad;
  return QN_OK;
}
extern "C" int qn_debug_eig3(qn_ctx* c, int which, const double* a6, uint32_t n, double* w_out, double* v_out) {
  if (!c || !a6 || !w_out || !v_out || which < 0 || which > 1 || n > QN_DEBUG_EIG3_MAX) return QN_ERR_INVALID_ARG;
  if (n == 0) return QN_OK;
  HIPCHK(c, hipSetDevice(c->device));
  double* d = nullptr;
  HIPCHK(c, hipMalloc(&d, 18 * (size_t)n * sizeof(double)));
  double* d_w = d + 6 * (size_t)n; double* d_v = d + 9 * (size_t)n;
  int rc = QN_OK;
  if (hipMemcpyAsync(d, a6, 6 * (size_t)n * sizeof(double), hipMemcpyHostToDevice, c->stream) != hipSuccess) rc = QN_ERR_HIP;
  if (rc == QN_OK) {
    hipLaunchKernelGGL(k_debug_eig3, dim3((n + QN_EIG3_DEBUG_BLOCK - 1) / QN_EIG3_DEBUG_BLOCK), dim3(QN_EIG3_DEBUG_BLOCK), 0, c->stream, which, (const double*)d, n, d_w, d_v);
    if (hipGetLastError() != hipSuccess || hipMemcpyAsync(w_out, d_w, 3 * (size_t)n * sizeof(double), hipMemcpyDeviceToHost, c->stream) != hipSuccess ||
        hipMemcpyAsync(v_out, d_v, 9 * (size_t)n * sizeof(double), hipMemcpyDeviceToHost, c->stream) != hipSuccess || hipStreamSynchronize(c->stream) != hipSuccess) rc = QN_ERR_HIP;
  }
  (void)hipFree(d);
  if (rc != QN_OK) { c->last_error = "debug_eig3: HIP call failed"; return rc; }
  return QN_OK;
}
namespace qn { hipError_t debug_launch_ldlt_solve6(const double* in, uint32_t n, double* out, hipStream_t stream); }
extern "C" int qn_debug_step_math(qn_ctx* c, int which, const double* in, uint32_t n, double* out) {
  static const uint32_t in_stride[QN_DEBUG_STEP_MATH_WHICH] = {43, 43, 59, 3, 9, 18}, out_stride[QN_DEBUG_STEP_MATH_WHICH] = {7, 6, 39, 9, 9, 3};
  if (!c || !in || !out || which < 0 || which >= QN_DEBUG_STEP_MATH_WHICH || n > QN_DEBUG_STEP_MATH_MAX) return QN_ERR_INVALID_ARG;
  if (n == 0) return QN_OK;
  HIPCHK(c, hipSetDevice(c->device));
  const size_t n_in = (size_t)in_stride[which] * n, n_out = (size_t)out_stride[which] * n;
// ... 147 lines not shown
      const uint32_t v = arg >> 24, cap = arg & 0xffffffu, fg = v == 0u ? 1u : (v == 3u ? 16u : 8u);
      if (n == 0 || n > QN_DEBUG_SEARCH_MAX_QUERIES || v > 3u || cap == 0 || cap > QN_DEBUG_SEARCH_MAX_RECORDED) return QN_ERR_INVALID_ARG;
      for (uint32_t i = 0; i < n; i++) {
        const uint32_t* r = in + 8 * (size_t)i;
        if (!finite_rec(r, 0, 4) || !(ds_f(r[3]) > 0.f)) return QN_ERR_INVALID_ARG;
      }
      w_in = 8 * (size_t)n; w_out = (((size_t)n * fg + 63) / 64) * 64 * (2 + (size_t)cap); break; }
    case QN_DS_LANE_BALL_KNN: default: {
      const uint32_t KM = arg & 63u, k = (arg >> 8) & 63u;
      if (n == 0 || n > QN_DEBUG_SEARCH_MAX_QUERIES || !kmax_ok(KM) || k < 1 || k > KM || (arg & 0xffffc0c0u)) return QN_ERR_INVALID_ARG;
      for (uint32_t i = 0; i < n; i++) {
        const uint32_t* r = in + 8 * (size_t)i;
        if (!finite_rec(r, 0, 4) || !(ds_f(r[3]) > 0.f)) return QN_ERR_INVALID_ARG;
      }
      w_in = 8 * (size_t)n; w_out = (size_t)(2 * k + 4) * n; break; }
  }
  if (w_in + w_out > QN_DEBUG_SEARCH_MAX_WORDS) return QN_ERR_INVALID_ARG;
  HIPCHK(c, hipSetDevice(c->device));
  uint32_t* dv = nullptr;
  HIPCHK(c, hipMalloc(&dv, (w_in + w_out + 2) * sizeof(uint32_t)));
  uint32_t* d_out = dv + ((w_in + 1) & ~(size_t)1);
  int rc = QN_OK;
  if ((w_in && hipMemcpyAsync(dv, in, w_in * sizeof(uint32_t), hipMemcpyHostToDevice, c->stream) != hipSuccess) || hipMemsetAsync(d_out, 0, w_out * sizeof(uint32_t), c->stream) != hipSuccess ||
      (which == QN_DS_DIVMOD && hipMemsetAsync(d_out + 4, 0xff, 8, c->stream) != hipSuccess)) rc = QN_ERR_HIP;
  if (rc == QN_OK) {
    if (qn::debug_launch_search(which, g, ncells, dv, n, arg, d_out, c->stream) != hipSuccess || hipMemcpyAsync(out_v, d_out, w_out * sizeof(uint32_t), hipMemcpyDeviceToHost, c->stream) != hipSuccess ||
        hipStreamSynchronize(c->stream) != hipSuccess) rc = QN_ERR_HIP;
  }
  (void)hipFree(dv);
  if (rc != QN_OK) { c->last_error = "debug_search: HIP call failed"; return rc; }
  return QN_OK;
}
extern "C" int qn_debug_get_counters(qn_ctx* c, uint32_t out[16]) {
  if (!c || !c->dbg_counters) return QN_ERR_INVALID_ARG;
  if (hipStreamSynchronize(c->stream) != hipSuccess) return QN_ERR_HIP;
  if (hipMemcpy(out, c->dbg_counters, 16 * sizeof(uint32_t), hipMemcpyDeviceToHost) != hipSuccess) return QN_ERR_HIP;
  return QN_OK;
}
extern "C" int qn_debug_get(qn_ctx* c, const char* key, double* value) {
  if (!c || !key || !value) return QN_ERR_INVALID_ARG;
  const std::string k(key);
  if (k == "verify_mismatches" || k == "verify_passes" || k == "verify_first") {
    if (!c->v_counters) return QN_ERR_NOT_READY;
    uint32_t h[4];
    if (hipStreamSynchronize(c->stream) != hipSuccess || hipMemcpy(h, c->v_counters, 16, hipMemcpyDeviceToHost) != hipSuccess) return QN_ERR_HIP;
    *value = k == "verify_mismatches" ? h[0] : (k == "verify_passes" ? h[1] : h[2]);
    return QN_OK;
  }
  if (k == "feat_mismatches" || k == "feat_verified" || k == "feat_first_mismatch") {
    if (!c->q_mm_vcnt) return QN_ERR_NOT_READY;
    uint32_t h[4];
    if (hipStreamSynchronize(c->stream) != hipSuccess || hipMemcpy(h, c->q_mm_vcnt, 16, hipMemcpyDeviceToHost) != hipSuccess) return QN_ERR_HIP;
    *value = k == "feat_mismatches" ? h[0] : (k == "feat_verified" ? h[2] : h[1]);
    return QN_OK;
  }
  if (k == "quatro_wall_features_ms") { *value = c->q_wall_ms[0]; return QN_OK; }
  if (k == "quatro_wall_match_ms") { *value = c->q_wall_ms[1]; return QN_OK; }
  if (k == "quatro_wall_solve_ms") { *value = c->q_wall_ms[2]; return QN_OK; }
  if (k == "extra_unseeded") { *value = c->last_extra_unseeded; return QN_OK; }
  if (k == "normals_width") { *value = c->quatro_normals_width(); return QN_OK; }
  if (k == "fpfh_width") { *value = c->quatro_fpfh_width(); return QN_OK; }
  if (k == "persist_launches") { *value = c->persist_launches; return QN_OK; }
  if (k == "persist_gave_up") { *value = c->persist_gave_up; return QN_OK; }
  if (k == "persist_fits") { *value = c->persist_fits ? 1 : 0; return QN_OK; }
  if (k == "persist_resident_blocks") { *value = c->persist_resident_blocks; return QN_OK; }
  if (k == "batch_launches") { *value = (double)c->batch_launches; return QN_OK; }
  if (k == "batch_pairs") { *value = (double)c->batch_pairs; return QN_OK; }
  if (k == "lanes_failed") { *value = c->lanes_failed ? 1.0 : 0.0; return QN_OK; }
  if (k == "batch_lanes") { *value = (double)c->knob.batch_lanes; return QN_OK; }
  if (k == "feat_fallbacks") { *value = c->feat_fallbacks; return QN_OK; }
  if (k == "feat_survivors") { *value = c->feat_survivors; return QN_OK; }
  return QN_ERR_INVALID_ARG;
}
extern "C" int qn_debug_get_clk(qn_ctx* c, unsigned long long* out , uint32_t* n) {
  if (!c || !out || !n || !c->clk_probe) return QN_ERR_INVALID_ARG;
  if (hipStreamSynchronize(c->stream) != hipSuccess || hipMemcpy(out, c->clk_probe, 8 * 8 * 256 + 8 * 12 * 1024, hipMemcpyDeviceToHost) != hipSuccess) return QN_ERR_HIP;
  *n = c->clk_n; return QN_OK;
}
extern "C" int qn_debug_get_list_probe(qn_ctx* c, unsigned long long* out ) {
  if (!c || !out || !c->list_probe) return QN_ERR_INVALID_ARG;
  if (hipStreamSynchronize(c->stream) != hipSuccess || hipMemcpy(out, c->list_probe, sizeof(unsigned long long) * 4 * 16384, hipMemcpyDeviceToHost) != hipSuccess) return QN_ERR_HIP;
  return QN_OK;
}
extern "C" int qn_debug_get_persist_clk(qn_ctx* c, unsigned long long* out ) {
  if (!c || !out || !c->pg_clk) return QN_ERR_INVALID_ARG;
  if (hipStreamSynchronize(c->stream) != hipSuccess || hipMemcpy(out, c->pg_clk, 8 * (64 * 16 + 16), hipMemcpyDeviceToHost) != hipSuccess) return QN_ERR_HIP;
  return QN_OK;
}
extern "C" int qn_debug_get_partials(qn_ctx* c, double* out , uint32_t* rows_per_buffer, double* state ) {
  if (!c || !out || !rows_per_buffer || !state) return QN_ERR_INVALID_ARG;
  *rows_per_buffer = QN_ACC_MAX_BLOCKS + 8;
  if (hipStreamSynchronize(c->stream) != hipSuccess || hipMemcpy(out, c->partials, 2 * sizeof(double) * (QN_ACC_MAX_BLOCKS + 8) * QN_NPART, hipMemcpyDeviceToHost) != hipSuccess
      || hipMemcpy(state, c->state, 2 * sizeof(GicpState), hipMemcpyDeviceToHost) != hipSuccess) return QN_ERR_HIP;
  return QN_OK;
}
extern "C" int qn_debug_get_grid(qn_ctx* c, int which, double out[8]) {
  if (!c || (which != 0 && which != 1) || !c->cloud[which].has_grid) return QN_ERR_INVALID_ARG;
  if (hipStreamSynchronize(c->stream) != hipSuccess || (c->stream2 && hipStreamSynchronize(c->stream2) != hipSuccess)) return QN_ERR_HIP;
  const GridDims& g = *c->cloud[which].dims_host;
  out[0] = g.ox; out[1] = g.oy; out[2] = g.oz; out[3] = g.cell; out[4] = g.nx; out[5] = g.ny; out[6] = g.nz; out[7] = g.eps;
  return QN_OK;
}

#include "qn_batch.inc"
#include "qn_quatro_host.inc"
#include "qn_kf_quatro.inc"
#include "qn_kf_submap.inc"
```

### fast-lio-sam-qn_amd/csrc/qn_gicp_kernels.cuh

```cuda
#pragma once
#include "qn_device.cuh"
#include "qn_step_math.cuh"
#include "qn_linearize.cuh"
#include "qn_knn_hist.cuh"
#include "../../include/qn_engine.h"
#include "qn_util_kernels.cuh"

namespace qn {

#define QN_ACC_MAX_BLOCKS 512
#define QN_MAX_TRACE 1024

struct GicpState {
  double x0[16], xi[16], delta[16];
  double H[36], b[6], d[6];
  double y0, yi, den;
  double lambda, nu;
  double final_H[36];
  double fitness;
  int outer, inner, phase, converged, lm_failed;
  uint32_t fb_count;
  uint32_t trace_len;
  uint32_t big_count;
  int pending;
// ... 362 lines not shown
    const uint32_t nq = LIST ? uni(*fb_count) : g.n;
    if (LIST && g.dbg && bx == 0 && threadIdx.x == 0) atomicAdd(&g.dbg[4], nq);
    const uint32_t wave0 = (LIST ? bx : xcd_block(bx, nbx)) * (QN_KNN_BLOCK / 64) + (threadIdx.x >> 6), nwaves = nbx * (QN_KNN_BLOCK / 64);
    for (uint32_t base = wave0 * 16; base < nq; base += nwaves * 16) {
      const uint32_t slot = base + (threadIdx.x & 15);
      bool active = slot < nq;
      uint32_t t = slot; float r = r0; bool general = false;
      if (LIST && active) { const uint2 rec = fb_list[slot]; t = rec.x; r = __uint_as_float(rec.y & 0x7fffffffu); general = (rec.y >> 31) != 0; }
      const float4 q = active ? g.pts[t] : make_float4(0, 0, 0, 0);
      const uint32_t i = __float_as_uint(q.w);
      int status = 2;
      {
        const int st = wave_knn_hist<HCAP, MM>(g, q.x, q.y, q.z, active && !general, r, k, max_rounds < 0 ? -max_rounds : max_rounds, my, knn_idx, knn_d2, i);
        if (!general) status = st;
      }
      if (!active || (threadIdx.x & 63) >= 16 || status == 0) continue;
      if (LIST) { const uint32_t fs = atomicAdd(gen_count, 1u); gen_list[fs] = make_uint2(t, __float_as_uint(r)); }
      else if (status == 2 || r > 2.5f * late_s(r0) || max_rounds < 0 ) { const uint32_t fs = atomicAdd(gen_count, 1u); gen_list[fs] = make_uint2(t, __float_as_uint(r)); }
      else { const uint32_t fs = atomicAdd(fb_count, 1u); fb_list[fs] = make_uint2(t, __float_as_uint(r)); }
    }
  }
};
template <bool LIST, int HCAP, bool MM = true>
__global__ void __launch_bounds__(QN_KNN_BLOCK, HCAP <= 32 ? 4 : 3) k_knn_hist(GridView g, int k, float r0, int max_rounds, int32_t* __restrict__ knn_idx, float* __restrict__ knn_d2,
                                                       uint2* __restrict__ fb_list, uint32_t* __restrict__ fb_count, uint2* __restrict__ gen_list, uint32_t* __restrict__ gen_count) {
  const KnnHistArgs a{g, k, r0, max_rounds, knn_idx, knn_d2, fb_list, fb_count, gen_list, gen_count};
  KnnHistK<LIST, HCAP, MM>::run(a, blockIdx.x, gridDim.x);
}

struct KnnSingleK {
  static constexpr int TB = QN_BLOCK, OCC = 1;
  struct Args { GridView g; int k; int32_t* knn_idx; float* knn_d2; const uint2* list; const uint32_t* count; uint2* gen_list; uint32_t* gen_count; };
  static __device__ __forceinline__ void run(const Args& a, const uint32_t bx, const uint32_t nbx) {
    __shared__ WaveLdsH1 lds[QN_BLOCK / 64];
    const GridView g = grid_resolve(a.g);
    const int k = a.k;
    int32_t* __restrict__ knn_idx = a.knn_idx; float* __restrict__ knn_d2 = a.knn_d2; const uint2* __restrict__ list = a.list; uint2* __restrict__ gen_list = a.gen_list; uint32_t* __restrict__ gen_count = a.gen_count;
    WaveLdsH1* my = &lds[threadIdx.x >> 6];
    const uint32_t nq = uni(*a.count);
    if (g.dbg && bx == 0 && threadIdx.x == 0) atomicAdd(&g.dbg[8], nq);
    const uint32_t wave0 = bx * (QN_BLOCK / 64) + (threadIdx.x >> 6), nwaves = nbx * (QN_BLOCK / 64);
    for (uint32_t e = wave0; e < nq; e += nwaves) {
      const uint2 rec = list[e];
      const float4 q = g.pts[rec.x];
      const uint32_t i = __float_as_uint(q.w);
      const int st = wave_knn_single(g, q.x, q.y, q.z, __uint_as_float(rec.y & 0x7fffffffu), k, my, knn_idx + (size_t)i * k, knn_d2 ? knn_d2 + (size_t)i * k : nullptr);
      if (st != 0 && (threadIdx.x & 63) == 0) { if (g.dbg) atomicAdd(&g.dbg[9], 1u); const uint32_t fs = atomicAdd(gen_count, 1u); gen_list[fs] = make_uint2(rec.x, rec.y & 0x7fffffffu); }
    }
  }
};
static __global__ void __launch_bounds__(QN_BLOCK) k_knn_single(GridView g, int k, int32_t* __restrict__ knn_idx, float* __restrict__ knn_d2,
                                                                const uint2* __restrict__ list, const uint32_t* __restrict__ count, uint2* __restrict__ gen_list, uint32_t* __restrict__ gen_count) {
  const KnnSingleK::Args a{g, k, knn_idx, knn_d2, list, count, gen_list, gen_count};
  KnnSingleK::run(a, blockIdx.x, gridDim.x);
}

template <int MODE>
__device__ __forceinline__ void xform_query(const float Tf[12], float x, float y, float z, float& qx, float& qy, float& qz) {
  if (MODE == 0) {
    qx = ((Tf[0] * x + Tf[1] * y) + Tf[2] * z) + Tf[3];
    qy = ((Tf[4] * x + Tf[5] * y) + Tf[6] * z) + Tf[7];
    qz = ((Tf[8] * x + Tf[9] * y) + Tf[10] * z) + Tf[11];
  } else {
    qx = Tf[0] * x + (Tf[1] * y + (Tf[2] * z + Tf[3]));
    qy = Tf[4] * x + (Tf[5] * y + (Tf[6] * z + Tf[7]));
    qz = Tf[8] * x + (Tf[9] * y + (Tf[10] * z + Tf[11]));
  }
}

__device__ __forceinline__ uint32_t late(uint32_t v) { asm volatile("" : "+v"(v)); return v; }
template <int MODE>
__device__ __forceinline__ void store_nn(unsigned long long key, uint32_t i, uint32_t t, double thr2, int32_t* __restrict__ corr, float* __restrict__ sqd, int32_t* __restrict__ nn_idx) {
  const float d2 = key_d2(key);
  if (MODE == 0) nn_idx[t] = key != QN_INF_KEY ? (int32_t)key_idx(key) : -1;
  if (MODE == 0) {
    const bool found = key != QN_INF_KEY;
    sqd[i] = found ? d2 : 0.f;
    corr[i] = (found && (double)d2 < thr2) ? (int32_t)key_idx(key) : -1;
  } else {
    sqd[i] = key != QN_INF_KEY ? d2 : __int_as_float(0x7f800000);
  }
}

struct NnOpt { float4* clear_ref; int cond; int group, group_min; unsigned long long* probe; uint32_t fb_small; };
struct NnSearchArgs { GridView src, tgt; const GicpState* st; double thr2; float r0; int max_rounds; int32_t* corr; float* sqd; int32_t* nn_idx; float4* nn_ref;
                      uint2* fb_list; uint32_t* fb_count; uint2* big_list; uint32_t* big_count; int big_blocks; float big_ratio; uint32_t* far_stats; NnOpt opt; };
template <int MODE, bool LIST, int BLOCK, bool GROUP = false>
struct NnSearchK {
  static constexpr int TB = BLOCK, OCC = GROUP ? 5 : 6;
  using Args = NnSearchArgs;
  static __device__ __forceinline__ void run(const Args& a, const uint32_t bx, const uint32_t nbx) {
    GridView src = a.src, tgt = a.tgt; const GicpState* __restrict__ st = a.st; const double thr2 = a.thr2; float r0 = a.r0; const int max_rounds = a.max_rounds;
    int32_t* __restrict__ corr = a.corr; float* __restrict__ sqd = a.sqd; int32_t* __restrict__ nn_idx = a.nn_idx; float4* __restrict__ nn_ref = a.nn_ref;
    uint2* __restrict__ fb_list = a.fb_list; uint32_t* __restrict__ fb_count = a.fb_count; uint2* __restrict__ big_list = a.big_list; uint32_t* __restrict__ big_count = a.big_count;
    const int big_blocks = a.big_blocks; const float big_ratio = a.big_ratio; uint32_t* __restrict__ far_stats = a.far_stats; const NnOpt opt = a.opt;

  __shared__ WaveLds lds[BLOCK / 64];
  if (MODE == 0 && uni(st->phase) != 0) return;
  if (MODE == 1 && uni(st->phase) != 2) return;
  if (opt.cond && !(uni(st->reserved) & opt.cond)) return;
  src = grid_resolve(src); tgt = grid_resolve(tgt); if (r0 < 0.f) r0 = -r0 * tgt.cell;
  __shared__ float sTf[12];
  if (threadIdx.x < 12) sTf[threadIdx.x] = (float)st->x0[threadIdx.x];
  __syncthreads();
  if (LIST && (int)bx >= (int)nbx - big_blocks) {
    const uint32_t nbig = uni(*big_count);
    if (tgt.dbg && bx == nbx - 1 && threadIdx.x == 0) atomicAdd(&tgt.dbg[7], nbig);
    uint32_t nfar = 0;
    const uint32_t bw0 = (bx - (nbx - big_blocks)) * (BLOCK / 64) + (threadIdx.x >> 6), nbw = big_blocks * (BLOCK / 64);
    const uint32_t E = (GROUP && opt.group && nbig >= (uint32_t)opt.group_min) ? min(16u, (nbig + (uint32_t)opt.group - 1u) / (uint32_t)opt.group) : 1u;
    if (GROUP && E > 1u) {
      const int lane = threadIdx.x & 63, qs = lane & 15;
      WaveLds* wl = &lds[threadIdx.x >> 6];
      const float INF = __int_as_float(0x7f800000);
      for (uint32_t w0 = bw0 * E; w0 < nbig; w0 += nbw * E) {
        const uint32_t slot = w0 + (uint32_t)qs;
        const bool active = (uint32_t)qs < E && slot < nbig;
        const uint2 rec = active ? big_list[slot] : make_uint2(0u, 0u);
        const float4 p = active ? src.pts[rec.x] : make_float4(0.f, 0.f, 0.f, 0.f);
        float qx, qy, qz; { float Tf[12];
#pragma unroll
          for (int j = 0; j < 12; j++) Tf[j] = sTf[j];
          xform_query<MODE>(Tf, p.x, p.y, p.z, qx, qy, qz); }
        const float v = __uint_as_float(rec.y);
        const float r = v > 0.f ? v * 1.1f + 0.5f * tgt.cell : -v;
        const bool finite_q = (qx - qx == 0.f) && (qy - qy == 0.f) && (qz - qz == 0.f) && (r - r == 0.f);
        unsigned long long key = QN_INF_KEY; float second = INF, d_unseen = INF;
        unsigned long long todo = __ballot(active);
        while (todo) {
          const int al = __ffsll((long long)todo) - 1;
          const float ax = rdlane(qx, al), ay = rdlane(qy, al), az = rdlane(qz, al), ar = rdlane(r, al);
          const bool afin = rdlane((int)finite_q, al) != 0;
          const bool open_q = (todo >> lane) & 1ull;
          const bool member = open_q && (qs == (al & 15) || (afin && finite_q && sqdist(qx, qy, qz, ax, ay, az) <= 0.25f * ar * ar));
          const unsigned long long mm = __ballot(member);
          if (__popcll(mm) <= 4) {
            unsigned long long k1; float s1, du1;
            wave_search_single(tgt, ax, ay, az, ar, INF, k1, s1, du1, wl);
            if (member) { key = k1; second = s1; d_unseen = du1; }
          } else {
            wave_search_far16(tgt, qx, qy, qz, member, r, key, second, d_unseen, wl);
          }
          todo &= ~mm;
        }
        if (active && lane < 16) {
          const uint32_t tl = late(rec.x);
          store_nn<MODE>(key, late(__float_as_uint(p.w)), tl, thr2, corr, sqd, nn_idx);
          if (MODE == 0) nn_ref[tl] = make_float4(qx, qy, qz, key != QN_INF_KEY ? sqrtf(key_d2(key)) : INF);
        }
        if (far_stats && MODE == 0) {
          const unsigned long long fm = __ballot(active && lane < 16 && key != QN_INF_KEY && key_d2(key) > 36.f * tgt.cell * tgt.cell);
          if (lane == 0) nfar += (uint32_t)__popcll(fm);
        }
      }
      if (far_stats && MODE == 0 && (threadIdx.x & 63) == 0 && nfar) atomicAdd(&far_stats[3], nfar);
      return;
    }
    unsigned long long pr_sum = 0, pr_max = 0, pr_a = 0, pr_b = 0; uint32_t pr_n = 0;
    const uint32_t nfb_all = uni(*fb_count);
    const uint32_t nfb1 = (opt.fb_small && nfb_all <= opt.fb_small) ? nfb_all : 0u;
    for (uint32_t w = bw0; w < nbig + nfb1; w += nbw) {
      const uint2 rec = w < nbig ? big_list[w] : fb_list[w - nbig];
      const float4 p = src.pts[rec.x];
      float qx, qy, qz; { float Tf[12];
#pragma unroll
          for (int j = 0; j < 12; j++) Tf[j] = sTf[j];
          xform_query<MODE>(Tf, p.x, p.y, p.z, qx, qy, qz); }
      const float v = __uint_as_float(rec.y);
      const float r = v > 0.f ? v * 1.1f + 0.5f * tgt.cell : -v;
      unsigned long long key; float second, d_unseen;
      const unsigned long long pt0 = opt.probe ? wall_clock64() : 0ull;
      SingleStats sst;
      wave_search_single(tgt, qx, qy, qz, r, __int_as_float(0x7f800000), key, second, d_unseen, &lds[threadIdx.x >> 6], sst, opt.probe != nullptr);
      if (opt.probe) { const unsigned long long dt = wall_clock64() - pt0; pr_sum += dt; pr_n++;
        if (dt > pr_max) { pr_max = dt; pr_a = ((unsigned long long)sst.rounds << 48) | ((unsigned long long)min(sst.segs, 0xffffffu) << 24) | (unsigned long long)min(sst.cand, 0xffffffu);
          pr_b = ((unsigned long long)__float_as_uint(sst.r_first) << 32) | __float_as_uint(key != QN_INF_KEY ? sqrtf(key_d2(key)) : -1.f); } }
      if ((threadIdx.x & 63) == 0) {
        const uint32_t tl = late(rec.x);
        store_nn<MODE>(key, late(__float_as_uint(p.w)), tl, thr2, corr, sqd, nn_idx);
        if (MODE == 0) nn_ref[tl] = make_float4(qx, qy, qz, fminf(sqrtf(second), d_unseen));
        if (key != QN_INF_KEY && key_d2(key) > 36.f * tgt.cell * tgt.cell) nfar++;
      }
    }
    if (far_stats && MODE == 0 && (threadIdx.x & 63) == 0 && nfar) atomicAdd(&far_stats[3], nfar);
    if (opt.probe && (threadIdx.x & 63) == 0 && bw0 < 16384u) { opt.probe[4 * bw0] = (pr_max << 32) | pr_n; opt.probe[4 * bw0 + 1] = pr_sum; opt.probe[4 * bw0 + 2] = pr_a; opt.probe[4 * bw0 + 3] = pr_b; }
    return;
  }
  const uint32_t nq = LIST ? uni(*fb_count) : src.n;
  if (LIST && opt.fb_small && nq <= opt.fb_small) return;
  if (LIST && tgt.dbg && bx == 0 && threadIdx.x == 0) atomicAdd(&tgt.dbg[5], nq);
  const uint32_t wave0 = bx * (BLOCK / 64) + (threadIdx.x >> 6), nwaves = (nbx - (LIST ? big_blocks : 0)) * (BLOCK / 64);
  for (uint32_t base = wave0 * 16; base < nq; base += nwaves * 16) {
    const uint32_t slot = base + (threadIdx.x & 15);
    const bool active = slot < nq;
    uint32_t t = slot; float r = r0, r_cap = __int_as_float(0x7f800000);
    if (LIST && active) {
      const uint2 rec = fb_list[slot]; t = rec.x;
      const float v = __uint_as_float(rec.y);
      if (v < 0.f) r = -v; else { r_cap = v; r = fminf(v, r0); }
    }
    const float4 p = active ? src.pts[t] : make_float4(0, 0, 0, 0);
    float qx, qy, qz; { float Tf[12];
#pragma unroll
          for (int j = 0; j < 12; j++) Tf[j] = sTf[j];
          xform_query<MODE>(Tf, p.x, p.y, p.z, qx, qy, qz); }
    Best1 sink; sink.init();
    float d_unseen;
    const bool cert = wave_search<4>(tgt, qx, qy, qz, active, r, r_cap, max_rounds, sink, &lds[threadIdx.x >> 6], d_unseen);
    const bool mine = active && (threadIdx.x & 48) == 0;
    const bool done = cert || LIST;
    if (!LIST && MODE == 0 && opt.clear_ref && mine) opt.clear_ref[t] = make_float4(0.f, 0.f, 0.f, 0.f);
    if (mine && done) {
      const uint32_t tl = late(t);
      store_nn<MODE>(sink.key, late(__float_as_uint(p.w)), tl, thr2, corr, sqd, nn_idx);
      if (MODE == 0) nn_ref[tl] = make_float4(qx, qy, qz, fminf(sqrtf(sink.second), d_unseen));
    }
    if (!LIST) {
      const float rn = r;
      const bool far = rn > big_ratio * r0;
      wave_append(big_list, big_count, mine && !done && far, make_uint2(t, __float_as_uint(-rn)));
      wave_append(fb_list, fb_count, mine && !done && !far, make_uint2(t, __float_as_uint(-rn)));
    }
  }
  }
};
template <int MODE, bool LIST, int BLOCK, bool GROUP = false>
__global__ void __launch_bounds__(BLOCK, GROUP ? 5 : 6) k_nn_search(GridView src, GridView tgt, const GicpState* __restrict__ st, double thr2, float r0, int max_rounds,
                                                        int32_t* __restrict__ corr, float* __restrict__ sqd, int32_t* __restrict__ nn_idx, float4* __restrict__ nn_ref,
                                                        uint2* __restrict__ fb_list, uint32_t* __restrict__ fb_count,
                                                        uint2* __restrict__ big_list, uint32_t* __restrict__ big_count, int big_blocks, float big_ratio, uint32_t* __restrict__ far_stats, NnOpt opt) {
  const NnSearchArgs a{src, tgt, st, thr2, r0, max_rounds, corr, sqd, nn_idx, nn_ref, fb_list, fb_count, big_list, big_count, big_blocks, big_ratio, far_stats, opt};
  NnSearchK<MODE, LIST, BLOCK, GROUP>::run(a, blockIdx.x, gridDim.x);
}


typedef __attribute__((address_space(1))) unsigned long long qn_gu64;
__device__ __forceinline__ void pr_store(unsigned long long* p, unsigned long long bits) { __hip_atomic_store((qn_gu64*)p, bits, __ATOMIC_RELAXED, __HIP_MEMORY_SCOPE_AGENT); }
__device__ __forceinline__ unsigned long long pr_load(const unsigned long long* p) { return __hip_atomic_load((qn_gu64*)p, __ATOMIC_RELAXED, __HIP_MEMORY_SCOPE_AGENT); }
__device__ __forceinline__ void row_store(double* p, double v, const bool coherent) {
  if (coherent) pr_store((unsigned long long*)p, (unsigned long long)__double_as_longlong(v)); else *p = v;
}

#define QN_LANE_ROWS 9
template <int MODE>
struct NnLaneK {
  static constexpr int TB = 256, OCC = 6;
  using Args = NnSearchArgs;
  static __device__ __forceinline__ void run(const Args& a, const uint32_t bx, const uint32_t) {
    const GicpState* __restrict__ st = a.st; const NnOpt opt = a.opt;
    if (MODE == 0 && uni(st->phase) != 0) return;
    if (MODE == 1 && uni(st->phase) != 2) return;
    if (opt.cond && !(uni(st->reserved) & opt.cond)) return;
    const GridView src = grid_resolve(a.src), tgt = grid_resolve(a.tgt);
    float r0 = a.r0; if (r0 < 0.f) r0 = -r0 * tgt.cell;
    float Tf[12];
#pragma unroll
    for (int j = 0; j < 12; j++) Tf[j] = uni((float)st->x0[j]);
    const uint32_t t = bx * TB + threadIdx.x;
    const bool active = t < src.n;
    const float4 p = active ? src.pts[t] : make_float4(0, 0, 0, 0);
    float qx, qy, qz; xform_query<MODE>(Tf, p.x, p.y, p.z, qx, qy, qz);
    if (MODE == 0 && opt.clear_ref && active) opt.clear_ref[t] = make_float4(0.f, 0.f, 0.f, 0.f);
    float r = r0;
    const int x0 = cell_coord(qx - r, tgt.ox, tgt.inv_cell, tgt.nx), x1 = cell_coord(qx + r, tgt.ox, tgt.inv_cell, tgt.nx);
    const int y0 = cell_coord(qy - r, tgt.oy, tgt.inv_cell, tgt.ny), y1 = cell_coord(qy + r, tgt.oy, tgt.inv_cell, tgt.ny);
    const int z0 = cell_coord(qz - r, tgt.oz, tgt.inv_cell, tgt.nz), z1 = cell_coord(qz + r, tgt.oz, tgt.inv_cell, tgt.nz);
    const int tx0 = x0 >> 3, ntr = (x1 >> 3) - tx0 + 1, nyr = y1 - y0 + 1, nzr = z1 - z0 + 1;
    const bool scan = active && nyr <= 3 && nzr <= 3 && ntr <= 2;
    Best1 sink; sink.init();
    const float4* __restrict__ pts = tgt.pts; const uint32_t* __restrict__ cs = tgt.cell_start;
    const uint32_t tile_zy = (uint32_t)tgt.nty * (uint32_t)tgt.ntx;
    uint32_t kz[3], ky[3];
#pragma unroll
    for (int d = 0; d < 3; d++) {
      const int z = z0 + d, y = y0 + d;
      kz[d] = (((uint32_t)(z >> 2) * tile_zy) << 7) | ((uint32_t)(z & 3) << 5);
      ky[d] = (((uint32_t)(y >> 2) * (uint32_t)tgt.ntx) << 7) | ((uint32_t)(y & 3) << 3);
    }
    const bool two = scan && ntr == 2;
    const int xb0 = min(x1, (tx0 << 3) + 7);
    const uint32_t kx0 = ((uint32_t)tx0 << 7) | (uint32_t)(x0 & 7), xlen0 = (uint32_t)(xb0 - x0) + 1u;
    const uint32_t kx1 = (uint32_t)(tx0 + 1) << 7, xlen1 = (uint32_t)(x1 - ((tx0 + 1) << 3)) + 1u;
    uint32_t s0[QN_LANE_ROWS], len0[QN_LANE_ROWS], off1[QN_LANE_ROWS], tot[QN_LANE_ROWS];
#pragma unroll
    for (int rr = 0; rr < QN_LANE_ROWS; rr++) {
      const int dz = rr / 3, dy = rr % 3;
      const bool rv = scan && dy < nyr && dz < nzr;
      uint32_t a0 = 0, b0 = 0, a1 = 0, b1 = 0;
      const uint32_t kr = kz[dz] + ky[dy];
      if (rv) { a0 = cs[kr + kx0]; b0 = cs[kr + kx0 + xlen0]; }
      if (rv && two) { a1 = cs[kr + kx1]; b1 = cs[kr + kx1 + xlen1]; }
      s0[rr] = a0; len0[rr] = b0 - a0; off1[rr] = a1 - len0[rr]; tot[rr] = len0[rr] + (b1 - a1);
    }
#pragma unroll
    for (int rr = 0; rr < QN_LANE_ROWS; rr++) {
      const uint32_t l0 = len0[rr], sa = s0[rr], sb = off1[rr], last = tot[rr] - 1u;
      for (uint32_t v = 0; v < tot[rr]; v += 4) {
        const uint32_t v1 = min(v + 1u, last), v2 = min(v + 2u, last), v3 = min(v + 3u, last);
        const float4 c0 = pts[v + (v < l0 ? sa : sb)], c1 = pts[v1 + (v1 < l0 ? sa : sb)], c2 = pts[v2 + (v2 < l0 ? sa : sb)], c3 = pts[v3 + (v3 < l0 ? sa : sb)];
        sink.consider<true>(true, sqdist(qx, qy, qz, c0.x, c0.y, c0.z), __float_as_uint(c0.w));
        sink.consider<true>(v + 1u <= last, sqdist(qx, qy, qz, c1.x, c1.y, c1.z), __float_as_uint(c1.w));
        sink.consider<true>(v + 2u <= last, sqdist(qx, qy, qz, c2.x, c2.y, c2.z), __float_as_uint(c2.w));
        sink.consider<true>(v + 3u <= last, sqdist(qx, qy, qz, c3.x, c3.y, c3.z), __float_as_uint(c3.w));
      }
    }
    const float INF = __int_as_float(0x7f800000);
    bool certified = false; float d_unseen = INF;
    if (scan) {
      float d = INF;
      if (x0 > 0) d = fminf(d, qx - (tgt.ox + x0 * tgt.cell));
      if (x1 < tgt.nx - 1) d = fminf(d, (tgt.ox + (x1 + 1) * tgt.cell) - qx);
      if (y0 > 0) d = fminf(d, qy - (tgt.oy + y0 * tgt.cell));
      if (y1 < tgt.ny - 1) d = fminf(d, (tgt.oy + (y1 + 1) * tgt.cell) - qy);
      if (z0 > 0) d = fminf(d, qz - (tgt.oz + z0 * tgt.cell));
      if (z1 < tgt.nz - 1) d = fminf(d, (tgt.oz + (z1 + 1) * tgt.cell) - qz);
      if (d == INF || !(r == r)) { certified = true; d_unseen = INF; }
      else { d -= tgt.eps; d_unseen = d; certified = d > 0.f && sink.full() && sink.worst_d2() < d * d; }
      if (!certified) r = sink.full() ? fmaxf(sqrtf(sink.worst_d2()) * 1.000001f + tgt.eps, r + tgt.eps) : 2.f * r + tgt.cell;
    }
    if (active && certified) {
      store_nn<MODE>(sink.key, __float_as_uint(p.w), t, a.thr2, a.corr, a.sqd, a.nn_idx);
      if (MODE == 0) a.nn_ref[t] = make_float4(qx, qy, qz, fminf(sqrtf(sink.second), d_unseen));
    }
    const bool far = r > a.big_ratio * r0;
    wave_append(a.big_list, a.big_count, active && !certified && far, make_uint2(t, __float_as_uint(-r)));
    wave_append(a.fb_list, a.fb_count, active && !certified && !far, make_uint2(t, __float_as_uint(-r)));
  }
};
template <int MODE>
__global__ void __launch_bounds__(256, 6) k_nn_lane(NnSearchArgs a) { NnLaneK<MODE>::run(a, blockIdx.x, gridDim.x); }


#define QN_TRACK_SEG 8
__device__ __forceinline__ bool track_bound_holds(float d0, float delta, float bound) {
  return (sqrtf(d0) + delta) * 1.000004f < bound;
}

static __global__ void k_reset_lists(GicpState* st) { if (threadIdx.x == 0 && blockIdx.x == 0) { st->fb_count = 0; st->big_count = 0; } }
static __global__ void k_verify_nn(uint32_t n, const GicpState* __restrict__ st, const int32_t* __restrict__ nn_a, const int32_t* __restrict__ nn_b,
                                   const float* __restrict__ sqd_a, const float* __restrict__ sqd_b, const int32_t* __restrict__ corr_a, const int32_t* __restrict__ corr_b,
                                   uint32_t* __restrict__ counters ) {
  if (st->phase != 0) return;
  const uint32_t t = blockIdx.x * blockDim.x + threadIdx.x;
  if (t == 0) atomicAdd(&counters[1], 1u);
  if (t >= n) return;
  bool bad = nn_a[t] != nn_b[t];
  if (sqd_a) bad = bad || __float_as_uint(sqd_a[t]) != __float_as_uint(sqd_b[t]) || corr_a[t] != corr_b[t];
  if (bad) { atomicAdd(&counters[0], 1u); atomicCAS(&counters[2], 0u, t + 1u); }
}


__device__ __forceinline__ void d_propose(GicpState* st, double lambda, SolveWork* A) {
  double Hl[36], rhs[6], dl[6];
#pragma unroll
  for (int i = 0; i < 6; i++)
#pragma unroll
    for (int j = 0; j < 6; j++) Hl[6 * i + j] = j <= i ? st->H[6 * i + j] : 0.0;
  if (!d_ldlt_solve6_fast(Hl, lambda, rhs, dl, st->b)) {
#pragma unroll
    for (int i = 0; i < 6; i++) A->rhs[i] = rhs[i];
    d_ldlt_solve6(st->H, lambda, st->d, A);
#pragma unroll
    for (int i = 0; i < 6; i++) dl[i] = st->d[i];
  }
  double R[3][3]; d_so3_exp(dl, R);
  double delta[16], xi[16];
#pragma unroll
  for (int i = 0; i < 16; i++) delta[i] = 0;
#pragma unroll
  for (int a = 0; a < 3; a++) {
#pragma unroll
    for (int b = 0; b < 3; b++) delta[4 * a + b] = R[a][b];
    delta[4 * a + 3] = dl[3 + a];
  }
  delta[15] = 1.0;
  double x0l[16];
#pragma unroll
  for (int i = 0; i < 16; i++) x0l[i] = st->x0[i];
  d_iso_mul(delta, x0l, xi);
#pragma unroll
  for (int i = 0; i < 6; i++) st->d[i] = dl[i];
#pragma unroll
  for (int i = 0; i < 16; i++) { st->delta[i] = delta[i]; st->xi[i] = xi[i]; }
}

__device__ inline void d_finish_outer(GicpState* st, const GicpConfig& cfg, qn_iter_trace* trace, qn_iter_trace tr) {
  bool conv = d_is_converged(st->delta, cfg, &tr.max_dR, &tr.max_dt);
  if (cfg.force_iterations > 0) conv = false;
  if (st->trace_len < QN_MAX_TRACE) { if (trace) trace[st->trace_len] = tr; st->trace_len++; }
  st->outer += 1;
  const int maxit = cfg.force_iterations > 0 ? cfg.force_iterations : cfg.max_iterations;
  if (conv) { st->converged = 1; st->phase = 2; }
  else if (st->outer >= maxit) { st->phase = 2; }
  else st->phase = 0;
}

__device__ inline void solve_controller(GicpState* st, const double* sums, const GicpConfig& cfg, qn_iter_trace* trace, int mode, int phase, SolveWork* Awork) {
  st->fb_count = 0; st->big_count = 0;
  const bool lin = (mode == 1) || (mode == 0 && phase == 0);
  if (lin) {
    int t = 0;
    for (int r = 0; r < 6; r++) for (int c = r; c < 6; c++, t++) { st->H[6 * r + c] = sums[t]; st->H[6 * c + r] = sums[t]; }
    for (int r = 0; r < 6; r++) st->b[r] = sums[21 + r];
    st->y0 = sums[27];
  } else {
    st->yi = sums[27];
  }
  if (mode != 0) return;

// ... 281 lines not shown
```

### fast-lio-sam-qn_amd/qn_amd/engine.py

```python
import ctypes as C
import math
import os
import numpy as np
from . import build as _build

QN_OK, QN_ERR_INVALID_ARG, QN_ERR_EMPTY_CLOUD, QN_ERR_CAPACITY, QN_ERR_NOT_READY, QN_ERR_HIP, QN_ERR_NO_DEVICE, QN_ERR_INTERNAL = range(8)
QN_SOURCE, QN_TARGET = 0, 1
QN_VERIFY_SRC, QN_VERIFY_DST, QN_VERIFY_COARSE, QN_VERIFY_FINAL = 0, 1, 2, 3
FLOAT_MAX = 3.4028234663852886e38
KERNEL_FAMILIES = ["grid_build", "knn_cov", "nn_search", "nn_fallback", "accumulate", "solve", "fitness", "transform",
                   "fpfh_normals", "fpfh_spfh", "fpfh_fpfh", "feat_match", "gn_tick_fused", "knn_select", "match_tail", "far_refresh", "align_persist"]


class GicpParams(C.Structure):
    _fields_ = [("k_correspondences", C.c_int32), ("max_iterations", C.c_int32), ("max_corr_dist", C.c_double),
                ("transformation_epsilon", C.c_double), ("rotation_epsilon", C.c_double), ("optimizer", C.c_int32),
                ("lm_max_iterations", C.c_int32), ("lm_init_lambda_factor", C.c_double), ("force_iterations", C.c_int32),
                ("ransac_iterations", C.c_int32), ("ransac_outlier_threshold", C.c_double),
                ("euclidean_fitness_epsilon", C.c_double)]


class GicpResult(C.Structure):
    _fields_ = [("T", C.c_float * 16), ("T64", C.c_double * 16), ("H", C.c_double * 36), ("fitness", C.c_double),
                ("iterations", C.c_int32), ("converged", C.c_int32), ("lm_failed", C.c_int32), ("reserved", C.c_int32)]
# ... 68 lines not shown
    def __del__(self):
        try:
            self.close()
        except Exception:
            pass

    def check(self, st):
        if st != QN_OK:
            raise EngineError(st, self._l.qn_status_str(st).decode() + ": " + self._l.qn_last_error(self.h).decode())

    @property
    def stream(self):
        return self._l.qn_ctx_stream(self.h)

    def synchronize(self):
        self.check(self._l.qn_ctx_synchronize(self.h))

    def debug_set(self, key, value):
        self.check(self._l.qn_debug_set(self.h, key.encode(), C.c_double(value)))

    def debug_get(self, key):
        v = C.c_double()
        self.check(self._l.qn_debug_get(self.h, key.encode(), C.byref(v)))
        return v.value

    def debug_eig3(self, which, a6):
        a = np.ascontiguousarray(a6, dtype=np.float64).reshape(-1, 6)
        n = len(a)
        if n == 0:
            a = np.zeros((1, 6))
        w = np.zeros((max(n, 1), 3)); V = np.zeros((max(n, 1), 3, 3))
        self._l.qn_debug_eig3.argtypes = [C.c_void_p, C.c_int, C.c_void_p, C.c_uint32, C.c_void_p, C.c_void_p]
        self.check(self._l.qn_debug_eig3(self.h, C.c_int(which), _p(a), C.c_uint32(n), _p(w), _p(V)))
        return w[:n], V[:n]

    STEP_MATH_STRIDES = ((43, 7), (43, 6), (59, 39), (3, 9), (9, 9), (18, 3))

    def debug_step_math(self, which, records):
        if not 0 <= which < len(self.STEP_MATH_STRIDES):
            raise ValueError("debug_step_math: which = %r" % (which,))
        si, so = self.STEP_MATH_STRIDES[which]
        a = np.ascontiguousarray(records, dtype=np.float64).reshape(-1, si)
        n = len(a)
        if n == 0:
            a = np.zeros((1, si))
        out = np.zeros((max(n, 1), so))
        self._l.qn_debug_step_math.argtypes = [C.c_void_p, C.c_int, C.c_void_p, C.c_uint32, C.c_void_p]
        self.check(self._l.qn_debug_step_math(self.h, C.c_int(which), _p(a), C.c_uint32(n), _p(out)))
        return out[:n]

    LIN_POINT, LIN_EMIT, LIN_ROWS = 0, 1, 2
    LIN_POINT_STRIDE, LIN_HEAD, LIN_LANE, LIN_BLOCK, LIN_NPART = 37, 25, 13, 256, 28

    def debug_linearize(self, which, data, arg=0):
        if which == self.LIN_POINT:
            si, shape = self.LIN_POINT_STRIDE, lambda n: (n, self.LIN_NPART)
        elif which == self.LIN_EMIT:
            if arg not in (1, 2, 3, 4):
                raise ValueError("debug_linearize: %r trips" % (arg,))
            si, shape = self.LIN_HEAD + arg * self.LIN_BLOCK * self.LIN_LANE, lambda n: (n, 5, self.LIN_NPART)
        elif which == self.LIN_ROWS:
            si, shape = self.LIN_NPART, lambda n: (min(n, 1) * self.LIN_NPART,)
        else:
            raise ValueError("debug_linearize: which = %r" % (which,))
        a = np.ascontiguousarray(data, dtype=np.float64).reshape(-1, si)
        n = len(a)
        if n == 0:
            a = np.zeros((1, si))
        out = np.zeros(max(int(np.prod(shape(n))), 1))
        self._l.qn_debug_linearize.argtypes = [C.c_void_p, C.c_int, C.c_void_p, C.c_uint32, C.c_uint32, C.c_void_p]
        self.check(self._l.qn_debug_linearize(self.h, C.c_int(which), _p(a), C.c_uint32(n), C.c_uint32(arg), _p(out)))
        return out[:int(np.prod(shape(n)))].reshape(shape(n))

    DS_DUMP, DS_BEST1, DS_BOUNDS, DS_DIVMOD, DS_STREAM_BOX, DS_WAVE_SEARCH1, DS_WAVE_SEARCH_SINGLE, DS_WAVE_SEARCH_FAR16, DS_BESTK, DS_WAVE_SEARCH_K, DS_LANE_BALL_KNN, DS_STREAM_CLUSTERS, DS_BALL_CELLS = range(13)

    def debug_search(self, which, grid, words, n, arg, n_out):
        a = np.ascontiguousarray(words, dtype=np.uint32).reshape(-1)
        if a.size == 0:
            a = np.zeros(1, dtype=np.uint32)
        out = np.zeros(max(int(n_out), 1), dtype=np.uint32)
        self._l.qn_debug_search.argtypes = [C.c_void_p, C.c_int, C.c_int, C.c_void_p, C.c_uint32, C.c_uint32, C.c_void_p]
        self.check(self._l.qn_debug_search(self.h, C.c_int(which), C.c_int(grid), _p(a), C.c_uint32(n), C.c_uint32(arg), _p(out)))
        return out[:int(n_out)]

    def grid_info(self, which):
        out = np.zeros(8)
        self.check(self._l.qn_debug_get_grid(self.h, C.c_int(which), _p(out)))
        return dict(origin=out[:3], cell=out[3], dims=out[4:7].astype(int), eps=out[7])

    def prof_enable(self, on=True):
        self.check(self._l.qn_prof_enable(self.h, C.c_int(1 if on else 0)))

    def prof_reset(self):
        self.check(self._l.qn_prof_reset(self.h))

    def prof_stats(self):
        out = {}
        for i, name in enumerate(KERNEL_FAMILIES):
            ks = KernelStat()
            self.check(self._l.qn_prof_get(self.h, C.c_int(i), C.byref(ks)))
            out[name] = (ks.total_ms, ks.launches)
        return out


def _cloud_arg(xyz):
    a = np.ascontiguousarray(xyz, dtype=np.float32)
    if a.ndim != 2 or a.shape[1] < 3:
        raise ValueError("cloud must be (n, >=3) float32")
    return a, a.shape[0], a.shape[1] * 4


class NanoGICP:

    def __init__(self, ctx):
        self.ctx = ctx
        self._l = ctx._l
        self.p = GicpParams()
        self._l.qn_gicp_default_params(C.byref(self.p))
        self._res = None
        self._n = [0, 0]
        self._push()

    def _push(self):
        self.ctx.check(self._l.qn_gicp_set_params(self.ctx.h, C.byref(self.p)))

    def bind(self):
        self._push()

    def setNumThreads(self, n):
        self.num_threads = n

    def setCorrespondenceRandomness(self, k):
        self.p.k_correspondences = k; self._push()

    def setMaximumIterations(self, n):
        self.p.max_iterations = n; self._push()

    def setRANSACIterations(self, n):
        self.p.ransac_iterations = n; self._push()

    def setMaxCorrespondenceDistance(self, d):
        self.p.max_corr_dist = d; self._push()

    def setTransformationEpsilon(self, e):
        self.p.transformation_epsilon = e; self._push()

    def setEuclideanFitnessEpsilon(self, e):
        self.p.euclidean_fitness_epsilon = e; self._push()

    def setRANSACOutlierRejectionThreshold(self, t):
        self.p.ransac_outlier_threshold = t; self._push()

    def setRotationEpsilon(self, e):
        self.p.rotation_epsilon = e; self._push()

    def setLMMaxIterations(self, n):
        self.p.lm_max_iterations = n; self._push()

    def setLMInitLambdaFactor(self, f):
        self.p.lm_init_lambda_factor = f; self._push()

    def setOptimizer(self, name):
        self.p.optimizer = 0 if name == "lm" else 1; self._push()

    def setForceIterations(self, n):
        self.p.force_iterations = n; self._push()
# ... 1453 lines not shown
```

### include/qn_engine.h

```cpp
#ifndef QN_ENGINE_H
#define QN_ENGINE_H

#include <stdint.h>

#ifdef __cplusplus
extern "C" {
#endif

typedef struct qn_ctx qn_ctx;

enum {
  QN_OK = 0,
  QN_ERR_INVALID_ARG = 1,
  QN_ERR_EMPTY_CLOUD = 2,
  QN_ERR_CAPACITY = 3,
  QN_ERR_NOT_READY = 4,
  QN_ERR_HIP = 5,
  QN_ERR_NO_DEVICE = 6,
  QN_ERR_INTERNAL = 7
};

enum { QN_SOURCE = 0, QN_TARGET = 1 };
enum { QN_OPT_LM = 0, QN_OPT_GN = 1 };

// ... 374 lines not shown
  double p[6];
} qn_sim_prim;
typedef struct {
  uint32_t n_beams, n_cols;
  const double *cos_el, *sin_el;
  const double *cos_az, *sin_az;
  double min_range, max_range, sigma;
} qn_sim_sensor;
int  qn_sim_lidar_to_store(qn_kf_store*, const qn_sim_prim* prims, uint32_t n_prims, const qn_sim_sensor* sensor, const double* poses16,
                           const uint32_t* seeds, uint32_t n_scans, int32_t* ids_out, uint32_t* n_out);

#define QN_SC_MAX_RINGS 64u
#define QN_SC_MAX_SECTORS 360u
#define QN_SC_MAX_BINS 8192u
#define QN_SC_MAX_PREFILTER 1024u
#define QN_SC_MAX_TOP_K 1024u
#define QN_SC_MAX_RESULTS (1u << 26)
typedef struct {
  uint32_t n_rings;
  uint32_t n_sectors;
  double max_radius;
  double lidar_height;
  uint32_t ringkey_prefilter;
  uint32_t pad_;
} qn_sc_params;
int  qn_kf_sc_set_params(qn_kf_store*, const qn_sc_params* p);
int  qn_kf_sc_get_params(qn_kf_store*, qn_sc_params* p);
int  qn_kf_sc_describe(qn_kf_store*, const int32_t* ids, uint32_t count);
int  qn_kf_sc_get(qn_kf_store*, int32_t id, float* desc , double* ringkey , double* colnorm );
int  qn_kf_sc_query(qn_kf_store*, const int32_t* query_ids, uint32_t nq, const double* stamps, uint32_t n_stamps, double tdiff, uint32_t top_k,
                    int32_t* ids_out, double* dist_out, int32_t* shift_out, uint32_t* n_out);

int  qn_gicp_get_covariances(qn_ctx*, int which, double* cov9_out);
int  qn_gicp_knn(qn_ctx*, int which, int k, int32_t* idx_out, float* d2_out);
int  qn_gicp_linearize(qn_ctx*, const double T[16], double H[36], double b[6], double* err,
                       int32_t* corr_out, float* sqd_out);
int  qn_gicp_compute_error(qn_ctx*, const double T[16], double* err);

int  qn_prof_enable(qn_ctx*, int on);
int  qn_prof_reset(qn_ctx*);
int  qn_prof_get(qn_ctx*, int kernel_family, qn_kernel_stat* out);
int  qn_debug_set(qn_ctx*, const char* key, double value);
int  qn_debug_get_counters(qn_ctx*, uint32_t out[16]);
int  qn_debug_selftest(qn_ctx*, uint32_t n_waves, uint32_t seed, uint32_t* mismatches);
#define QN_DEBUG_EIG3_MAX (1u << 24)
int  qn_debug_eig3(qn_ctx*, int which, const double* a6, uint32_t n, double* w_out, double* v_out);
#define QN_DEBUG_STEP_MATH_WHICH 6
#define QN_DEBUG_STEP_MATH_MAX (1u << 20)
int  qn_debug_step_math(qn_ctx*, int which, const double* in, uint32_t n, double* out);
#define QN_DEBUG_LINEARIZE_WHICH 3
#define QN_DEBUG_LINEARIZE_MAX_POINTS (1u << 20)
#define QN_DEBUG_LINEARIZE_MAX_BLOCKS (1u << 11)
#define QN_DEBUG_LINEARIZE_MAX_ROWS (1u << 16)
int  qn_debug_linearize(qn_ctx*, int which, const double* in, uint32_t n, uint32_t arg, double* out);
#define QN_DEBUG_SEARCH_WHICH 13
#define QN_DS_DUMP 0
#define QN_DS_BEST1 1
#define QN_DS_BOUNDS 2
#define QN_DS_DIVMOD 3
#define QN_DS_STREAM_BOX 4
#define QN_DS_WAVE_SEARCH1 5
#define QN_DS_WAVE_SEARCH_SINGLE 6
#define QN_DS_WAVE_SEARCH_FAR16 7
#define QN_DS_BESTK 8
#define QN_DS_WAVE_SEARCH_K 9
#define QN_DS_LANE_BALL_KNN 10
#define QN_DS_STREAM_CLUSTERS 11
#define QN_DS_BALL_CELLS 12
#define QN_DEBUG_SEARCH_MAX_WAVES (1u << 12)
#define QN_DEBUG_SEARCH_MAX_QUERIES (1u << 16)
#define QN_DEBUG_SEARCH_MAX_STEPS 64u
#define QN_DEBUG_SEARCH_MAX_RECORDED (1u << 16)
#define QN_DEBUG_SEARCH_MAX_WORDS (1u << 26)
int  qn_debug_search(qn_ctx*, int which, int grid, const void* in, uint32_t n, uint32_t arg, void* out);
#define QN_DEBUG_MAP_PRIMS_WHICH 9
#define QN_DEBUG_MAP_PRIMS_MAX_BLOCKS (1u << 16)
#define QN_DEBUG_MAP_PRIMS_MAX_NODES (1u << 20)
#define QN_DEBUG_MAP_PRIMS_MAX_EDGES (1u << 20)
int  qn_kf_debug_map_prims(qn_kf_store*, int which, const void* in, uint32_t n, uint32_t arg, void* out);
int  qn_debug_get(qn_ctx*, const char* key, double* value);
int  qn_debug_get_grid(qn_ctx*, int which, double out[8]);
int  qn_debug_get_partials(qn_ctx*, double* out, uint32_t* rows_per_buffer, double* state);
int  qn_debug_get_list_probe(qn_ctx*, unsigned long long* out );
int  qn_debug_get_persist_clk(qn_ctx*, unsigned long long* out );
int  qn_debug_get_clk(qn_ctx*, unsigned long long* out , uint32_t* n);

#ifdef __cplusplus
}
#endif
#endif
```

Baseline: 4534.

## Write NN leftover lists into per-block regions instead of global atomic appends

```diff
diff --git a/fast-lio-sam-qn_amd/csrc/qn_batch.inc b/fast-lio-sam-qn_amd/csrc/qn_batch.inc
--- a/fast-lio-sam-qn_amd/csrc/qn_batch.inc
+++ b/fast-lio-sam-qn_amd/csrc/qn_batch.inc
@@ -63,7 +63,7 @@
 struct ScratchSwap {
   qn_ctx* c;
   static void sw(qn_ctx* c) {
-    std::swap(c->scan_sums, c->scan_sums2); std::swap(c->fb_list, c->fb_list2); std::swap(c->big_list, c->big_list2); std::swap(c->fb_count2, c->fb_count2b);
+    std::swap(c->scan_sums, c->scan_sums2); std::swap(c->fb_list, c->fb_list2); std::swap(c->big_list, c->big_list2); std::swap(c->fb_count2, c->fb_count2b); std::swap(c->list_cnt, c->list_cnt2);
     std::swap(c->knn_idx, c->knn_idx2); std::swap(c->bbox_acc, c->bbox_acc2); std::swap(c->scan_status, c->scan_status2); std::swap(c->staging, c->staging2); std::swap(c->pin_up, c->pin_up2);
   }
   explicit ScratchSwap(qn_ctx* c_) : c(c_) { sw(c); }
@@ -253,6 +253,7 @@
           lane_push(v_acc, prep_accumulate(c, 0, true), nb);
           c->count_far_now = false;
         }
+        for (auto* v : {&v_g, &v_l}) for (auto& e : *v) if (e.a.opt.region_shift != (lane ? 8u : 6u)) e.a.opt.regions = 0u;
         if (lane) plan.add<NnLaneK<0>>(v_g, QN_K_NN_SEARCH); else plan.add<NnSearchK<0, false, QN_NN_BLOCK>>(v_g, QN_K_NN_SEARCH);
         if (group) plan.add<NnSearchK<0, true, QN_BLOCK, true>>(v_l, QN_K_NN_FALLBACK); else plan.add<NnSearchK<0, true, QN_BLOCK>>(v_l, QN_K_NN_FALLBACK);
         plan.add<AccumulateK>(v_acc, QN_K_ACCUMULATE);
diff --git a/fast-lio-sam-qn_amd/csrc/qn_context.h b/fast-lio-sam-qn_amd/csrc/qn_context.h
--- a/fast-lio-sam-qn_amd/csrc/qn_context.h
+++ b/fast-lio-sam-qn_amd/csrc/qn_context.h
@@ -26,6 +26,7 @@
   double cell_override = 0.0;
   int far_group = -1;
   bool far_ranked = true;
+  int list_regions = 1024;
   int nn_lane = -1;
   int track_from_tick = 3;
   int knn_mm = 1;
@@ -85,6 +86,8 @@
   int32_t* corr = nullptr; int32_t* nn_idx = nullptr; int32_t* knn_idx = nullptr; float4* nn_ref = nullptr; double* nrm_s_sorted = nullptr; qn::TargetRec* tgt_rec = nullptr; float* sqd = nullptr; float* sqd_fit = nullptr;
   int32_t* far_cand = nullptr; float4* far_cand_ref = nullptr; float2* far_cand_b = nullptr; unsigned long long* far_req = nullptr; uint32_t* far_stats = nullptr; double* far_rows = nullptr; int far_mode = 2;
   uint2* fb_list = nullptr; uint2* big_list = nullptr; uint32_t* fb_count2 = nullptr;
+  uint32_t* list_cnt = nullptr;
+  const qn::GicpState* dbg_list_st = nullptr; uint32_t dbg_list_regions = 0, dbg_list_shift = 0;
   float4* aligned = nullptr; bool aligned_valid = false;
   double* pose_tmp = nullptr; float* guess_tmp = nullptr;
   qn::ResultBlock* result_host = nullptr; double* scalar_host = nullptr;
@@ -101,7 +104,7 @@
   float* q_mean = nullptr; double* q_mean_psum = nullptr; void* q_host = nullptr;
   int unseeded_until = 3; bool count_far_now = false; int last_extra_unseeded = 0;
   hipStream_t stream2 = nullptr; hipEvent_t ev_pair = nullptr; bool pair_failed = false, tgt_on_stream2 = false, tgt_pending = false, no_pipe = false;
-  uint32_t* scan_sums2 = nullptr; uint2* fb_list2 = nullptr; uint2* big_list2 = nullptr; uint32_t* fb_count2b = nullptr; int32_t* knn_idx2 = nullptr;
+  uint32_t* scan_sums2 = nullptr; uint2* fb_list2 = nullptr; uint2* big_list2 = nullptr; uint32_t* fb_count2b = nullptr; uint32_t* list_cnt2 = nullptr; int32_t* knn_idx2 = nullptr;
   unsigned long long* pg_rows = nullptr; unsigned long long* pg_bc = nullptr; unsigned long long* pg_fit = nullptr; uint32_t* pg_status = nullptr; uint32_t* pg_status_host = nullptr;
   unsigned long long* pg_clk = nullptr; uint32_t pg_epoch = 0; bool persist_fits = true; int persist_resident_blocks = 0; uint32_t persist_launches = 0, persist_gave_up = 0;
   uint32_t* dbg_counters = nullptr;
diff --git a/fast-lio-sam-qn_amd/csrc/qn_device.cuh b/fast-lio-sam-qn_amd/csrc/qn_device.cuh
--- a/fast-lio-sam-qn_amd/csrc/qn_device.cuh
+++ b/fast-lio-sam-qn_amd/csrc/qn_device.cuh
@@ -543,7 +543,7 @@
       sink.consider(mine && in_tile && ccid == cid, sqdist(qx, qy, qz, cp.x, cp.y, cp.z), __float_as_uint(cp.w));
     });
     sink.template finish<S>(mine);
-    if (g.dbg && lane == 0) { atomicAdd(&g.dbg[0], (uint32_t)ncl); atomicAdd(&g.dbg[1], ncand); }
+    if (g.dbg && lane == 0) { atomicAdd(&g.dbg[0], (uint32_t)ncl); atomicAdd(&g.dbg[1], ncand); atomicAdd(&g.dbg[6], 1u); }
     bool retry = false;
     if (mine) {
       const int* b = lds->box[cid];
diff --git a/fast-lio-sam-qn_amd/csrc/qn_engine.hip b/fast-lio-sam-qn_amd/csrc/qn_engine.hip
--- a/fast-lio-sam-qn_amd/csrc/qn_engine.hip
+++ b/fast-lio-sam-qn_amd/csrc/qn_engine.hip
@@ -136,6 +136,7 @@
     sl.take(c->fb_list, sizeof(uint2) * max_points);
     sl.take(c->big_list, sizeof(uint2) * max_points);
     sl.take(c->fb_count2, 4 * sizeof(uint32_t));
+    sl.take(c->list_cnt, 2 * QN_LIST_REGIONS * sizeof(uint32_t));
     sl.take(c->aligned, sizeof(float4) * max_points);
     sl.take(c->pose_tmp, sizeof(double) * 16);
     sl.take(c->guess_tmp, sizeof(float) * 16);
@@ -143,6 +144,7 @@
     sl.take(c->fb_list2, sizeof(uint2) * max_points);
     sl.take(c->big_list2, sizeof(uint2) * max_points);
     sl.take(c->fb_count2b, 4 * sizeof(uint32_t));
+    sl.take(c->list_cnt2, 2 * QN_LIST_REGIONS * sizeof(uint32_t));
     sl.take(c->knn_idx2, sizeof(int32_t) * (size_t)max_points * 32);
     sl.take(c->staging2, (size_t)max_points * 32);
     sl.take(c->bbox_acc, 2 * (QN_BBOX_MAX_BLOCKS + 1) * sizeof(BBoxAcc)); c->bbox_acc2 = c->bbox_acc ? c->bbox_acc + (QN_BBOX_MAX_BLOCKS + 1) : nullptr;
@@ -259,7 +261,7 @@
 }
 static void swap_scratch(qn_ctx* c) {
   std::swap(c->stream, c->stream2); std::swap(c->scan_sums, c->scan_sums2); std::swap(c->fb_list, c->fb_list2); std::swap(c->big_list, c->big_list2);
-  std::swap(c->fb_count2, c->fb_count2b); std::swap(c->knn_idx, c->knn_idx2);
+  std::swap(c->fb_count2, c->fb_count2b); std::swap(c->list_cnt, c->list_cnt2); std::swap(c->knn_idx, c->knn_idx2);
   std::swap(c->bbox_acc, c->bbox_acc2); std::swap(c->scan_status, c->scan_status2);
   std::swap(c->pin_up, c->pin_up2);
   std::swap(c->staging, c->staging2);
@@ -459,11 +461,17 @@
   constexpr uint32_t LIST_SMALL = 6000;
   opt.fb_small = (mode == 0 && !c->knob.persist_batch_off) ? LIST_SMALL : 0u;
   NnOpt opt0; opt0.clear_ref = nullptr; opt0.cond = 0; opt0.group = 0; opt0.group_min = 0; opt0.probe = nullptr; opt0.fb_small = 0;
+  const bool lane = (c->lane.nn_lane > 0 || (c->lane.nn_lane < 0 && c->knob.persist_batch_off)) && mode == 0;
+  const uint32_t grid_nb = lane ? (S.n + 255u) / 256u : nb;
+  const bool regions = grid_nb * ((mode == 0 && opt.fb_small) ? 2u : 1u) <= (uint32_t)std::min(c->lane.list_regions, QN_LIST_REGIONS);
+  opt.list_cnt = opt0.list_cnt = c->list_cnt;
+  opt.regions = opt0.regions = regions ? grid_nb : 0u; opt.region_shift = opt0.region_shift = lane ? 8u : 6u;
+  if (mode == 0) { c->dbg_list_st = st; c->dbg_list_regions = opt.regions; c->dbg_list_shift = opt.region_shift; }
   if (mode == 0) c->clear_far_now = false;
   const NnOpt& o = mode == 0 ? opt : opt0;
   NnLaunch L;
-  L.lane = (c->lane.nn_lane > 0 || (c->lane.nn_lane < 0 && c->knob.persist_batch_off)) && mode == 0;
-  L.grid_nb = L.lane ? (S.n + 255u) / 256u : nb; L.list_nb = fbb + (uint32_t)big_blocks; L.group = mode == 0 && opt.group > 0;
+  L.lane = lane;
+  L.grid_nb = grid_nb; L.list_nb = fbb + (uint32_t)big_blocks; L.group = mode == 0 && opt.group > 0;
   L.grid = NnSearchArgs{S.grid, T.grid, st, thr2, NN_R0, 1, c->corr, sqd_out, c->nn_idx, c->nn_ref, c->fb_list, fbc, c->big_list, bgc, 0, NN_BIG_RATIO, far_stats, o};
   L.list = NnSearchArgs{S.grid, T.grid, st, thr2, NN_R0, 64, c->corr, sqd_out, c->nn_idx, c->nn_ref, c->fb_list, fbc, c->big_list, bgc, big_blocks, NN_BIG_RATIO, far_stats, o};
   return L;
@@ -1089,6 +1097,7 @@
   else if (k == "batch_trace") c->knob.batch_trace = v != 0;
   else if (k == "batch_member") c->knob.persist_batch_off = v != 0;
   else if (k == "knn_hist") c->knob.knn_hist = v != 0;
+  else if (k == "list_regions") c->lane.list_regions = std::max(0, std::min((int)v, QN_LIST_REGIONS));
   else if (k == "nn_lane") c->lane.nn_lane = v < 0 ? -1 : (v != 0 ? 1 : 0);
   else if (k == "track_from_tick") c->lane.track_from_tick = v < 1 ? 1 : (int)v;
   else if (k == "single_from_tick") c->knob.single_from_tick = v < 1 ? 1 : (int)v;
@@ -1402,6 +1411,25 @@
   if (hipStreamSynchronize(c->stream) != hipSuccess || hipMemcpy(out, c->list_probe, sizeof(unsigned long long) * 4 * 16384, hipMemcpyDeviceToHost) != hipSuccess) return QN_ERR_HIP;
   return QN_OK;
 }
+extern "C" int qn_debug_get_lists(qn_ctx* c, uint32_t* fb_out, uint32_t* n_fb, uint32_t* big_out, uint32_t* n_big, uint32_t* regions) {
+  if (!c || !fb_out || !n_fb || !big_out || !n_big || !regions || !c->dbg_list_st || !c->cloud[0].has_grid) return QN_ERR_INVALID_ARG;
+  const uint32_t n = c->cloud[0].n, nreg = c->dbg_list_regions, sh = c->dbg_list_shift;
+  GicpState hs; std::vector<uint32_t> cnt(2 * QN_LIST_REGIONS); std::vector<uint2> lst(n); std::vector<float4> pts(n);
+  if (hipStreamSynchronize(c->stream) != hipSuccess || hipMemcpy(&hs, c->dbg_list_st, sizeof(GicpState), hipMemcpyDeviceToHost) != hipSuccess
+      || hipMemcpy(cnt.data(), c->list_cnt, sizeof(uint32_t) * 2 * QN_LIST_REGIONS, hipMemcpyDeviceToHost) != hipSuccess
+      || hipMemcpy(pts.data(), c->cloud[0].sorted, sizeof(float4) * n, hipMemcpyDeviceToHost) != hipSuccess) return QN_ERR_HIP;
+  *regions = nreg;
+  for (int w = 0; w < 2; w++) {
+    const uint32_t total = w == 0 ? hs.fb_count : hs.big_count; const uint32_t* rc = cnt.data() + (w == 0 ? nreg : 0u); uint32_t* out = w == 0 ? fb_out : big_out; uint32_t m = 0;
+    if (total > n || hipMemcpy(lst.data(), w == 0 ? c->fb_list : c->big_list, sizeof(uint2) * n, hipMemcpyDeviceToHost) != hipSuccess) return QN_ERR_HIP;
+    auto emit = [&](const uint2 e) { out[3 * m] = e.x; out[3 * m + 1] = e.y; uint32_t i = 0xffffffffu; if (e.x < n) memcpy(&i, &pts[e.x].w, 4); out[3 * m + 2] = i; m++; };
+    if (nreg == 0) { for (uint32_t e = 0; e < total; e++) emit(lst[e]); }
+    else for (uint32_t g = 0; g < nreg; g++) for (uint32_t j = 0; j < rc[g] && m < n && ((size_t)g << sh) + j < n; j++) emit(lst[((size_t)g << sh) + j]);
+    if (m != total) { c->last_error = "list read-back: the region counts do not add up to the list's total"; return QN_ERR_HIP; }
+    *(w == 0 ? n_fb : n_big) = m;
+  }
+  return QN_OK;
+}
 extern "C" int qn_debug_get_persist_clk(qn_ctx* c, unsigned long long* out ) {
   if (!c || !out || !c->pg_clk) return QN_ERR_INVALID_ARG;
   if (hipStreamSynchronize(c->stream) != hipSuccess || hipMemcpy(out, c->pg_clk, 8 * (64 * 16 + 16), hipMemcpyDeviceToHost) != hipSuccess) return QN_ERR_HIP;
diff --git a/fast-lio-sam-qn_amd/csrc/qn_gicp_kernels.cuh b/fast-lio-sam-qn_amd/csrc/qn_gicp_kernels.cuh
--- a/fast-lio-sam-qn_amd/csrc/qn_gicp_kernels.cuh
+++ b/fast-lio-sam-qn_amd/csrc/qn_gicp_kernels.cuh
@@ -468,7 +468,59 @@
   }
 }
 
-struct NnOpt { float4* clear_ref; int cond; int group, group_min; unsigned long long* probe; uint32_t fb_small; };
+struct NnOpt { float4* clear_ref; int cond; int group, group_min; unsigned long long* probe; uint32_t fb_small; uint32_t* list_cnt; uint32_t regions, region_shift; };
+#define QN_LIST_REGIONS 1024
+template <int NW>
+__device__ __forceinline__ void region_append(const NnOpt& opt, uint2* __restrict__ fb_list, uint32_t* __restrict__ fb_total, uint2* __restrict__ big_list, uint32_t* __restrict__ big_total,
+                                              const uint32_t bx, const bool want_fb, const bool want_big, const uint2 rec, uint32_t (*wcnt)[2]) {
+  const int lane = threadIdx.x & 63, wid = threadIdx.x >> 6;
+  const unsigned long long mf = __ballot(want_fb), mb = __ballot(want_big);
+  if (lane == 0) { wcnt[wid][0] = (uint32_t)__popcll(mf); wcnt[wid][1] = (uint32_t)__popcll(mb); }
+  __syncthreads();
+  uint32_t of = 0, ob = 0, tf = 0, tb = 0;
+#pragma unroll
+  for (int w = 0; w < NW; w++) { const uint32_t cf = wcnt[w][0], cb = wcnt[w][1]; if (w < wid) { of += cf; ob += cb; } tf += cf; tb += cb; }
+  const unsigned long long below = (1ull << lane) - 1ull;
+  const uint32_t r0s = bx << opt.region_shift;
+  if (want_fb) fb_list[r0s + of + (uint32_t)__popcll(mf & below)] = rec;
+  if (want_big) big_list[r0s + ob + (uint32_t)__popcll(mb & below)] = rec;
+  if (threadIdx.x == 0) {
+    opt.list_cnt[bx] = tb; opt.list_cnt[opt.regions + bx] = tf;
+    if (tf) atomicAdd(fb_total, tf);
+    if (tb) atomicAdd(big_total, tb);
+  }
+}
+template <int BLOCK>
+__device__ __forceinline__ void region_prefix(const uint32_t* __restrict__ cnt, const uint32_t nreg, uint32_t* pre, uint32_t* wsum) {
+  constexpr int PER = QN_LIST_REGIONS / BLOCK;
+  static_assert(PER * BLOCK == QN_LIST_REGIONS && BLOCK % 64 == 0, "the block covers the count table in one pass");
+  const uint32_t b0 = threadIdx.x * PER;
+  uint32_t v[PER], s = 0;
+#pragma unroll
+  for (int j = 0; j < PER; j++) { v[j] = b0 + j < nreg ? cnt[b0 + j] : 0u; s += v[j]; }
+  uint32_t inc = s;
+  const int lane = threadIdx.x & 63, wid = threadIdx.x >> 6;
+#pragma unroll
+  for (int o = 1; o < 64; o <<= 1) { const uint32_t u = __shfl_up(inc, o); if (lane >= o) inc += u; }
+  if (lane == 63) wsum[wid] = inc;
+  __syncthreads();
+  uint32_t run = inc - s;
+  for (int w = 0; w < wid; w++) run += wsum[w];
+#pragma unroll
+  for (int j = 0; j < PER; j++) { if (b0 + j < nreg) pre[b0 + j] = run; run += v[j]; }
+  __syncthreads();
+}
+__device__ __forceinline__ uint32_t region_find(const uint32_t* pre, const uint32_t nrow, const uint32_t e, uint32_t& j) {
+  uint32_t g = 0;
+#pragma unroll
+  for (uint32_t step = QN_LIST_REGIONS / 2; step; step >>= 1) { const uint32_t c = g + step; if (c < nrow && pre[c] <= e) g = c; }
+  j = e - pre[g];
+  return g;
+}
+__device__ __forceinline__ uint32_t region_slot(const uint32_t* pre, const uint32_t nreg, const uint32_t shift, const uint32_t e) {
+  uint32_t j; const uint32_t g = region_find(pre, nreg, e, j);
+  return (g << shift) + j;
+}
 struct NnSearchArgs { GridView src, tgt; const GicpState* st; double thr2; float r0; int max_rounds; int32_t* corr; float* sqd; int32_t* nn_idx; float4* nn_ref;
                       uint2* fb_list; uint32_t* fb_count; uint2* big_list; uint32_t* big_count; int big_blocks; float big_ratio; uint32_t* far_stats; NnOpt opt; };
 template <int MODE, bool LIST, int BLOCK, bool GROUP = false>
@@ -482,6 +534,8 @@
     const int big_blocks = a.big_blocks; const float big_ratio = a.big_ratio; uint32_t* __restrict__ far_stats = a.far_stats; const NnOpt opt = a.opt;
 
   __shared__ WaveLds lds[BLOCK / 64];
+  __shared__ uint32_t s_pre[LIST ? QN_LIST_REGIONS : 1];
+  __shared__ uint32_t s_wsum[BLOCK / 64][2];
   if (MODE == 0 && uni(st->phase) != 0) return;
   if (MODE == 1 && uni(st->phase) != 2) return;
   if (opt.cond && !(uni(st->reserved) & opt.cond)) return;
@@ -495,6 +549,15 @@
     uint32_t nfar = 0;
     const uint32_t bw0 = (bx - (nbx - big_blocks)) * (BLOCK / 64) + (threadIdx.x >> 6), nbw = big_blocks * (BLOCK / 64);
     const uint32_t E = (GROUP && opt.group && nbig >= (uint32_t)opt.group_min) ? min(16u, (nbig + (uint32_t)opt.group - 1u) / (uint32_t)opt.group) : 1u;
+    const uint32_t nfb_all = uni(*fb_count);
+    const uint32_t nfb1 = (opt.fb_small && nfb_all <= opt.fb_small) ? nfb_all : 0u;
+    const uint32_t nreg = opt.regions, rshift = opt.region_shift;
+    if (nreg) {
+      const uint32_t first = (bx - (nbx - big_blocks)) * (BLOCK / 64);
+      const bool grouped = GROUP && E > 1u;
+      if (grouped ? first * E >= nbig : first >= nbig + nfb1) return;
+      region_prefix<BLOCK>(opt.list_cnt, (!grouped && nfb1) ? 2u * nreg : nreg, s_pre, &s_wsum[0][0]);
+    }
     if (GROUP && E > 1u) {
       const int lane = threadIdx.x & 63, qs = lane & 15;
       WaveLds* wl = &lds[threadIdx.x >> 6];
@@ -502,7 +565,7 @@
       for (uint32_t w0 = bw0 * E; w0 < nbig; w0 += nbw * E) {
         const uint32_t slot = w0 + (uint32_t)qs;
         const bool active = (uint32_t)qs < E && slot < nbig;
-        const uint2 rec = active ? big_list[slot] : make_uint2(0u, 0u);
+        const uint2 rec = active ? big_list[nreg ? region_slot(s_pre, nreg, rshift, slot) : slot] : make_uint2(0u, 0u);
         const float4 p = active ? src.pts[rec.x] : make_float4(0.f, 0.f, 0.f, 0.f);
         float qx, qy, qz; { float Tf[12];
 #pragma unroll
@@ -543,10 +606,10 @@
       return;
     }
     unsigned long long pr_sum = 0, pr_max = 0, pr_a = 0, pr_b = 0; uint32_t pr_n = 0;
-    const uint32_t nfb_all = uni(*fb_count);
-    const uint32_t nfb1 = (opt.fb_small && nfb_all <= opt.fb_small) ? nfb_all : 0u;
     for (uint32_t w = bw0; w < nbig + nfb1; w += nbw) {
-      const uint2 rec = w < nbig ? big_list[w] : fb_list[w - nbig];
+      uint32_t ws = w < nbig ? w : w - nbig;
+      if (nreg) { uint32_t j; const uint32_t g = region_find(s_pre, nfb1 ? 2u * nreg : nreg, w, j); ws = ((g < nreg ? g : g - nreg) << rshift) + j; }
+      const uint2 rec = w < nbig ? big_list[ws] : fb_list[ws];
       const float4 p = src.pts[rec.x];
       float qx, qy, qz; { float Tf[12];
 #pragma unroll
@@ -576,12 +639,18 @@
   if (LIST && opt.fb_small && nq <= opt.fb_small) return;
   if (LIST && tgt.dbg && bx == 0 && threadIdx.x == 0) atomicAdd(&tgt.dbg[5], nq);
   const uint32_t wave0 = bx * (BLOCK / 64) + (threadIdx.x >> 6), nwaves = (nbx - (LIST ? big_blocks : 0)) * (BLOCK / 64);
+  const uint32_t nreg = opt.regions, rshift = opt.region_shift;
+  if (LIST && nreg) {
+    if (bx * (BLOCK / 4) >= nq) return;
+    region_prefix<BLOCK>(opt.list_cnt + nreg, nreg, s_pre, &s_wsum[0][0]);
+  }
+  bool want_fb = false, want_big = false; uint2 left = make_uint2(0u, 0u);
   for (uint32_t base = wave0 * 16; base < nq; base += nwaves * 16) {
     const uint32_t slot = base + (threadIdx.x & 15);
     const bool active = slot < nq;
     uint32_t t = slot; float r = r0, r_cap = __int_as_float(0x7f800000);
     if (LIST && active) {
-      const uint2 rec = fb_list[slot]; t = rec.x;
+      const uint2 rec = fb_list[nreg ? region_slot(s_pre, nreg, rshift, slot) : slot]; t = rec.x;
       const float v = __uint_as_float(rec.y);
       if (v < 0.f) r = -v; else { r_cap = v; r = fminf(v, r0); }
     }
@@ -604,10 +673,14 @@
     if (!LIST) {
       const float rn = r;
       const bool far = rn > big_ratio * r0;
-      wave_append(big_list, big_count, mine && !done && far, make_uint2(t, __float_as_uint(-rn)));
-      wave_append(fb_list, fb_count, mine && !done && !far, make_uint2(t, __float_as_uint(-rn)));
-    }
-  }
+      if (nreg) { want_big = mine && !done && far; want_fb = mine && !done && !far; left = make_uint2(t, __float_as_uint(-rn)); }
+      else {
+        wave_append(big_list, big_count, mine && !done && far, make_uint2(t, __float_as_uint(-rn)));
+        wave_append(fb_list, fb_count, mine && !done && !far, make_uint2(t, __float_as_uint(-rn)));
+      }
+    }
+  }
+  if (!LIST && nreg) region_append<BLOCK / 64>(opt, fb_list, fb_count, big_list, big_count, bx, want_fb, want_big, left, s_wsum);
   }
 };
 template <int MODE, bool LIST, int BLOCK, bool GROUP = false>
@@ -709,8 +782,13 @@
       if (MODE == 0) a.nn_ref[t] = make_float4(qx, qy, qz, fminf(sqrtf(sink.second), d_unseen));
     }
     const bool far = r > a.big_ratio * r0;
-    wave_append(a.big_list, a.big_count, active && !certified && far, make_uint2(t, __float_as_uint(-r)));
-    wave_append(a.fb_list, a.fb_count, active && !certified && !far, make_uint2(t, __float_as_uint(-r)));
+    if (opt.regions) {
+      __shared__ uint32_t s_wcnt[TB / 64][2];
+      region_append<TB / 64>(opt, a.fb_list, a.fb_count, a.big_list, a.big_count, bx, active && !certified && !far, active && !certified && far, make_uint2(t, __float_as_uint(-r)), s_wcnt);
+    } else {
+      wave_append(a.big_list, a.big_count, active && !certified && far, make_uint2(t, __float_as_uint(-r)));
+      wave_append(a.fb_list, a.fb_count, active && !certified && !far, make_uint2(t, __float_as_uint(-r)));
+    }
   }
 };
 template <int MODE>
diff --git a/fast-lio-sam-qn_amd/qn_amd/engine.py b/fast-lio-sam-qn_amd/qn_amd/engine.py
--- a/fast-lio-sam-qn_amd/qn_amd/engine.py
+++ b/fast-lio-sam-qn_amd/qn_amd/engine.py
@@ -174,6 +174,13 @@
         self._l.qn_debug_search.argtypes = [C.c_void_p, C.c_int, C.c_int, C.c_void_p, C.c_uint32, C.c_uint32, C.c_void_p]
         self.check(self._l.qn_debug_search(self.h, C.c_int(which), C.c_int(grid), _p(a), C.c_uint32(n), C.c_uint32(arg), _p(out)))
         return out[:int(n_out)]
+
+    def leftover_lists(self, n_source):
+        fb = np.zeros(3 * max(int(n_source), 1), dtype=np.uint32); big = np.zeros_like(fb)
+        nf, nb, reg = C.c_uint32(), C.c_uint32(), C.c_uint32()
+        self._l.qn_debug_get_lists.argtypes = [C.c_void_p, C.c_void_p, C.c_void_p, C.c_void_p, C.c_void_p, C.c_void_p]
+        self.check(self._l.qn_debug_get_lists(self.h, _p(fb), C.byref(nf), _p(big), C.byref(nb), C.byref(reg)))
+        return fb[:3 * nf.value].reshape(-1, 3).copy(), big[:3 * nb.value].reshape(-1, 3).copy(), int(reg.value)
 
     def grid_info(self, which):
         out = np.zeros(8)
diff --git a/include/qn_engine.h b/include/qn_engine.h
--- a/include/qn_engine.h
+++ b/include/qn_engine.h
@@ -480,7 +480,8 @@
 int  qn_debug_get_grid(qn_ctx*, int which, double out[8]);
 int  qn_debug_get_partials(qn_ctx*, double* out, uint32_t* rows_per_buffer, double* state);
 int  qn_debug_get_list_probe(qn_ctx*, unsigned long long* out );
-int  qn_debug_get_persist_clk(qn_ctx*, unsigned long long* out );
+int  qn_debug_get_lists(qn_ctx*, uint32_t* fb_out, uint32_t* n_fb, uint32_t* big_out, uint32_t* n_big, uint32_t* regions);
+int  qn_debug_get_persist_clk(qn_ctx*,unsigned long long* out );
 int  qn_debug_get_clk(qn_ctx*, unsigned long long* out , uint32_t* n);
 
 #ifdef __cplusplus
```

Result: no change. 4514 (median of 2 runs) (-0.4%).
